# acerbilab/gpyreg

Hardware: AMD Instinct MI355X
Metric: GP-fits/sec (NLL+grad, N=4096 D=10) (higher is better)
Workload: dtype f64

## Files before the change

### gpyreg_amd/_lib.py

```python

from __future__ import annotations

import ctypes as C
import os
import threading

import numpy as np

_HERE = os.path.dirname(os.path.abspath(__file__))
LIB_PATH = os.environ.get("GPYREG_AMD_LIB") or os.path.join(_HERE, "lib", "libgpcore.so")

K_SE, K_MATERN, K_RQ, K_SE_ISO, K_MATERN_ISO = range(5)
F64, F32 = 0, 1
KLO_ZERO, KLO_ROW, KLO_COL = 0, 1, 2
KHI_FULL, KHI_ROW, KHI_COL = 0, 1, 2
CV_LOSSES = {"lpd": 0, "mse": 1}

_dp = C.c_void_p
_ip = C.c_void_p
_vp = C.c_void_p
_dpp = C.POINTER(C.c_double)

SIGNATURES = {
    "gpc_create": (C.c_int, [C.c_int, C.POINTER(_vp)]),
# ... 24 lines not shown
    "gpc_nll_batch_K": (
        C.c_int,
        [_vp, C.c_int, C.c_int, C.c_int, _dp, _vp, _vp, _dp, _dp, C.c_int, C.c_int, _dp, C.c_int, _dp,
         C.c_int, _dp, _dp, _dp, _ip, _ip],
    ),
    "gpc_posterior_batch_K": (
        C.c_int, [_vp, C.c_int, C.c_int, _dp, _dp, _dp, C.c_int, C.POINTER(_vp), _dp, _ip, _ip]),
    "gpc_predict_K": (C.c_int, [_vp, C.c_int, _dp, _dp, _dp, _dp, _dp]),
    "gpc_set_data_gobs": (C.c_int, [_vp, _dp, _dp, C.c_int, C.c_int, _dp, _dp, C.c_int]),
    "gpc_posterior_batch_gobs": (
        C.c_int, [_vp, C.c_int, C.c_int, C.c_int, C.c_int, _dp, _dp, _dp, C.POINTER(_vp), _dp, _dp, _ip, _ip]),
    "gpc_nll_batch_gobs": (C.c_int, [_vp, C.c_int, C.c_int, C.c_int, C.c_int, _dp, _dp, _dp, _dp, _dp, _ip, _ip]),
    "gpc_predict_gobs": (C.c_int, [_vp, _dp, C.c_int, _dp, _dp]),
    "gpc_debug_gobs_cov": (C.c_int, [_vp, C.c_int, C.c_int, _dp, _dp, C.c_int, C.c_int, _dp, C.c_int, _dp]),
    "gpc_debug_gobs_cross": (
        C.c_int, [_vp, C.c_int, C.c_int, _dp, _dp, C.c_int, C.c_int, _dp, C.c_int, _dp, C.c_int, _dp, _dp, _dp]),
    "gpc_post_fetch": (C.c_int, [_vp, C.c_int, _dp, _dp, _dp]),
    "gpc_post_free": (C.c_int, [_vp]),
    "gpc_predict": (C.c_int, [_vp, _dp, C.c_int, _dp, _dp]),
    "gpc_predict_grad": (C.c_int, [_vp, _dp, C.c_int, _dp, _dp, _dp, _dp]),
    "gpc_grad_post": (C.c_int, [_vp, _dp, C.c_int, C.c_int, _dp, _dp, _dp]),
    "gpc_predict_hess": (C.c_int, [_vp, _dp, C.c_int, C.c_int, _dp, _dp, _dp, _dp, _dp, _dp]),
    "gpc_nll_hess": (C.c_int, [_vp, _dp, C.c_int, _dp, C.c_int, C.c_int, _dp, _dp, _dp, _dp]),
    "gpc_cv_grad": (C.c_int, [_vp, C.c_int, _dp, _dp, _dp, _dp, _dp, _dp, _dp]),
    "gpc_predict_hyp_grad": (
        C.c_int, [_vp, _dp, C.c_int, C.c_int, _dp, _dp, C.c_int, C.c_int, _dp, C.c_int, _dp, _dp, _dp, _dp]),
    "gpc_post_append": (C.c_int, [_vp, _dp, _dp, C.c_double, _ip]),
    "gpc_post_recompute": (C.c_int, [_vp, C.c_int, _ip, _dp, _dp, _dp, C.c_int, _dp, _ip, _ip]),
    "gpc_post_append_K": (C.c_int, [_vp, _dp, _dp, _dp, _dp, C.c_double, _ip]),
    "gpc_post_append_block": (C.c_int, [_vp, C.c_int, _dp, _dp, _dp, _ip]),
    "gpc_post_append_block_K": (C.c_int, [_vp, C.c_int, _dp, _dp, _dp, _dp, _dp, _ip]),
    "gpc_post_remove": (C.c_int, [_vp, C.c_int, _ip, _dp, _ip]),
    "gpc_debug_remove_panel": (C.c_int, [_vp, C.c_int, C.c_int, _dp, _dp, _dp, _dp]),
    "gpc_debug_remove_apply": (C.c_int, [_vp, C.c_int, C.c_int, C.c_int, C.c_int, C.c_int, _dp, _dp, _dp]),
    "gpc_post_recompute_K": (C.c_int, [_vp, C.c_int, _ip, _dp, _dp, _dp, C.c_int, _dp, _ip, _ip]),
    "gpc_predict_full": (C.c_int, [_vp, _dp, C.c_int, _dp, _dp]),
    "gpc_predict_cov": (C.c_int, [_vp, _dp, C.c_int, _dp, C.c_int, _dp, C.c_int, _dp, _dp, _dp]),
    "gpc_lookahead_batch": (C.c_int, [_vp, _dp, C.c_int, _dp, C.c_int, _dp, C.c_int, _dp, C.c_int, _ip, _dp]),
    "gpc_draw": (C.c_int, [_vp, _dp, C.c_int, C.c_int, C.c_ulonglong, C.c_int, _dp, _dp, _dp]),
    "gpc_paths_create": (C.c_int, [_vp, C.c_int, C.c_int, C.c_ulonglong, C.c_int, _dp, _dp, C.POINTER(_vp)]),
    "gpc_paths_eval": (C.c_int, [_vp, _dp, C.c_int, _dp, _dp]),
    "gpc_paths_free": (C.c_int, [_vp]),
    "gpc_debug_paths_fetch": (C.c_int, [_vp, C.c_int, _dp, _dp, _dp, _dp]),
    "gpc_quad": (C.c_int, [_vp, _dp, _dp, C.c_int, C.c_int, _dp, _dp]),
    "gpc_quad_grad": (C.c_int, [_vp, _dp, _dp, C.c_int, C.c_int, _dp, _dp, _dp, _dp, _dp, _dp]),
    "gpc_quad_cov": (C.c_int, [_vp, _dp, _dp, C.c_int, _dp, _dp]),
    "gpc_quad_mix": (C.c_int, [_vp, _dp, _dp, _dp, C.c_int, C.c_int, C.c_int] + [_dp] * 10),
    "gpc_cv": (C.c_int, [_vp, C.c_int, _ip, _ip, _dp, _dp, _dp, _dp, _ip]),
    "gpc_last_timing": (C.c_int, [_vp, _dp, _dp]),
    "gpc_last_lauum_timing": (C.c_int, [_vp, _dp, _dp]),
    "gpc_set_option": (C.c_int, [_vp, C.c_char_p, C.c_int]),
    "gpc_get_option": (C.c_int, [_vp, C.c_char_p, _ip]),
    "gpc_mfma_peak": (C.c_int, [_vp, C.c_int, _dp, _dp, _dp]),
    "gpc_debug_gemm": (
        C.c_int,
        [_vp, C.c_int, C.c_int, C.c_int, C.c_int, C.c_int, C.c_int, C.c_double, C.c_int, C.c_int,
         C.c_int, C.c_int, _dp, _dp, _dp],
    ),
    "gpc_debug_leaf": (C.c_int, [_vp, C.c_int, _dp, _dp, _dp, _dp, _ip]),
    "gpc_debug_factor": (C.c_int, [_vp, C.c_int, C.c_int, _dp, _dp, _dp, _dp, _dp, _ip]),
    "gpc_debug_factor_plan": (C.c_int, [_vp] + [C.c_int] * 7 + [_dp] * 7 + [_ip]),
    "gpc_debug_cov": (
        C.c_int,
        [_vp, C.c_int, C.c_int, C.c_int, C.c_int, _dp, C.c_double, C.c_double, _dp, _dp, C.c_int, C.c_int, _dp,
         C.c_int, _dp, _dp, _dp, _dp, _dp],
    ),
    "gpc_debug_blas1": (C.c_int, [_vp, C.c_int, C.c_int, _ip, _vp, _vp, _vp, _vp]),
    "gpc_debug_block_gram": (C.c_int, [_vp, C.c_int, C.c_int, C.c_int, C.c_int, _dp, _dp, C.c_int, _dp]),
    "gpc_debug_hess_contract": (
        C.c_int, [_vp, C.c_int, C.c_int, C.c_int, _dp, _dp, C.c_int, C.c_int, _dp, C.c_int, _dp, _dp, _dp, _dp]),
    "gpc_debug_hyp_cross": (
        C.c_int, [_vp, C.c_int, C.c_int, _dp, _dp, C.c_int, C.c_int, _dp, C.c_int, _dp, _dp, C.c_int, _dp, _dp]),
    "gpc_debug_nll_plane": (
        C.c_int, [_vp, C.c_int, C.c_int, _dp, _dp, C.c_int, C.c_int, C.c_int, _dp, _dp, _dp, _dp, _dp]),
    "gpc_debug_nll_d2": (C.c_int, [_vp, C.c_int, C.c_int, _dp, _dp, C.c_int, C.c_int, _dp, _dp, _dp]),
    "gpc_debug_nll_gram": (C.c_int, [_vp, C.c_int, C.c_int, _dp, _dp]),
    "gpc_debug_cv_trace": (C.c_int, [_vp, C.c_int, C.c_int, _dp, _dp, C.c_int, C.c_int, _dp, _dp, _dp, _dp, _dp]),
    "gpc_debug_cv_weights": (C.c_int, [_vp, C.c_int, C.c_int, _dp, _dp, _dp, _dp, _dp]),
    "gpc_debug_normals": (C.c_int, [_vp, C.c_ulonglong, C.c_int, C.c_int, C.c_int, C.c_int, C.c_int, _dp]),
    "gpc_debug_workspace_hash": (C.c_int, [_vp, C.c_int, C.c_int, C.c_int, _vp]),
    "gpc_debug_chunk_plan": (C.c_int, [C.c_int, C.c_ulonglong, C.c_ulonglong, C.c_ulonglong, C.c_int]),
    "gpc_debug_scratch_bytes": (C.c_int, [C.c_char_p, C.c_int, _ip, C.c_int, _vp, _vp, _ip]),
    "gpc_debug_gemm_queues": (C.c_int, [C.c_int] * 8 + [_ip] * 4),
    "gpc_debug_gemm_form": (
        C.c_int,
        [_vp, C.c_int, C.c_int, C.c_int, C.c_int, C.c_int, C.c_int, _vp, _vp, _dp, C.c_longlong, _dp, _dp, _ip, _ip],
    ),
}
EXPERIMENT_SIGNATURES = {
    "gpc_debug_dag": (C.c_int, [C.c_int, C.c_int, C.c_int, C.c_int, _ip, _ip, _dp, _ip, C.c_int, C.c_int]),
}
EXPERIMENTS_LIB_PATH = os.path.join(_HERE, "lib", "libgpcore_exp.so")

DK_PLANE_FN = C.CFUNCTYPE(C.c_int, _vp, C.c_int, C.c_int, _dpp)


class _GemmProductStruct(C.Structure):
    _fields_ = ([(n, C.c_int) for n in ("M", "N", "K", "a_kmajor", "b_kmajor", "beta", "klo", "khi", "lower_only",
                                        "lda", "ldb", "ldc")]
                + [(n, C.c_longlong) for n in ("off_a", "off_b", "off_c", "s_a", "s_b", "s_c", "size_a", "size_b",
                                               "size_c")]
                + [("alpha", C.c_double), ("A", _vp), ("B", _vp), ("C", _vp)])


class GemmProduct:

    def __init__(self, A, B, C, M, N, K, a_kmajor=0, b_kmajor=0, alpha=1.0, beta=0, klo=0, khi=0, lower_only=0,
                 lda=None, ldb=None, ldc=None, off_a=0, off_b=0, off_c=0, s_a=0, s_b=0, s_c=0):
        self.A, self.B, self.C = _f64(A).ravel(), _f64(B).ravel(), _f64(C).ravel()
        self.M, self.N, self.K = int(M), int(N), int(K)
        self.a_kmajor, self.b_kmajor = int(bool(a_kmajor)), int(bool(b_kmajor))
        self.alpha, self.beta, self.klo, self.khi, self.lower_only = float(alpha), int(beta), klo, khi, int(bool(lower_only))
        self.lda = int(lda if lda is not None else (M if a_kmajor else K))
        self.ldb = int(ldb if ldb is not None else (N if b_kmajor else K))
        self.ldc = int(ldc if ldc is not None else N)
        self.off_a, self.off_b, self.off_c = int(off_a), int(off_b), int(off_c)
        self.s_a, self.s_b, self.s_c = int(s_a), int(s_b), int(s_c)


BLAS1 = {name: code for code, name in enumerate((
    "trmv", "trmv_low", "gemv_sub", "trmv_t_part", "trmv_t_part_low", "trmv_t_sum", "dot", "mat_t_vec", "grad_tail",
    "colsum_prod", "colsum_vec", "diagq", "trace_plane", "extract", "neg_sym", "pad_load", "pad_rect", "load_K",
    "rect_copy", "grow_copy", "append_row", "append_low"))}
BLAS1_GUARD = 128

FORMS = {"plain": 0, "persist": 1, "persist_reserved": 2, "dual": 3, "colsq": 4, "wsq": 5}

_lib = None
_lock = threading.RLock()


def load():
    global _lib
    with _lock:
        if _lib is None:
            if not os.path.exists(LIB_PATH):
                raise RuntimeError(
                    f"{LIB_PATH} is missing: the HIP extension has not been built "
                    "(run `python -c 'import __graft_entry__ as g; g.build()'`). "
                    "gpyreg_amd has no CPU fallback."
                )
            lib = C.CDLL(LIB_PATH)
            for name, (res, args) in SIGNATURES.items():
                fn = getattr(lib, name)
                fn.restype = res
                fn.argtypes = args
            for name, (res, args) in EXPERIMENT_SIGNATURES.items():
                fn = getattr(lib, name, None)
                if fn is not None:
                    fn.restype = res
                    fn.argtypes = args
            _lib = lib
    return _lib


def is_experiments_build() -> bool:
    return hasattr(load(), "gpc_debug_dag")


def _f64(a):
    return np.ascontiguousarray(a, dtype=np.float64)


def _ptr(a):
    if a is None:
        return None
# ... 939 lines not shown
            ptr[1:] = np.cumsum([len(f) for f in folds])
            idx = np.ascontiguousarray(np.concatenate([np.asarray(f).ravel() for f in folds]), dtype=np.int32)
        n_out = F if F else N
        quad, logdet = np.empty((n_out, S)), np.empty((n_out, S))
        info = np.empty((n_out, S), dtype=np.int32)
        rc = self.ctx._lib.gpc_cv(self._h, F, _ptr(ptr), _ptr(idx), _ptr(dmu), _ptr(s2), _ptr(quad), _ptr(logdet),
                                  _ptr(info))
        self.ctx._check(rc, "gpc_cv")
        return dmu, s2, quad, logdet, info

    @_serial
    def free(self):
        if self._h:
            self.ctx._lib.gpc_post_free(self._h)
            self._h = None

    def __del__(self):
        try:
            if self.ctx._h:
                self.free()
        except Exception:
            pass


class Paths:

    def __init__(self, ctx: Context, h, S: int, N: int, D: int, R: int, F: int):
        self.ctx, self._h, self.S, self.N, self.D, self.R, self.F = ctx, h, S, N, D, R, F

    @_serial
    def eval(self, x_star, compute_grad=False):
        if not self._h:
            raise ValueError("paths: the handle has been closed")
        xs = _f64(x_star)
        if xs.ndim != 2 or xs.shape[1] != self.D:
            raise ValueError(f"paths: x_star must be (M, {self.D}), got {xs.shape}")
        M = xs.shape[0]
        f = np.empty((M, self.R, self.S))
        df = np.empty((M, self.D, self.R, self.S)) if compute_grad else None
        rc = self.ctx._lib.gpc_paths_eval(self._h, _ptr(xs), M, _ptr(f), _ptr(df))
        self.ctx._check(rc, "gpc_paths_eval")
        return (f, df) if compute_grad else f

    @_serial
    def fetch(self, s):
        theta, b = np.empty((self.F, self.D)), np.empty(self.F)
        wt, v = np.empty((self.F, self.R)), np.empty((self.N, self.R))
        rc = self.ctx._lib.gpc_debug_paths_fetch(self._h, int(s), _ptr(theta), _ptr(b), _ptr(wt), _ptr(v))
        self.ctx._check(rc, "gpc_debug_paths_fetch")
        return theta, b, wt, v

    @_serial
    def free(self):
        if self._h:
            self.ctx._lib.gpc_paths_free(self._h)
            self._h = None

    def __del__(self):
        try:
            if self.ctx._h:
                self.free()
        except Exception:
            pass


def gemm_queues(ntiles, batch, flags, tiles_m=0, tiles_n=0, klo=0, khi=0, lower_only=0, want_tiles=False,
                want_xcd=False):
    lib = load()
    n = int(ntiles) * int(batch)
    q_total = np.zeros(8, dtype=np.int32)
    q_items = np.full((max(n, 1), 2), -1, dtype=np.int32)
    tiles = np.full((ntiles, 2), -1, dtype=np.int32) if want_tiles else None
    xcd = np.full((batch, ntiles, 2), -1, dtype=np.int32) if want_xcd else None
    rc = lib.gpc_debug_gemm_queues(int(ntiles), int(batch), int(flags), int(tiles_m), int(tiles_n), int(klo), int(khi),
                                   int(bool(lower_only)), q_total.ctypes.data, q_items.ctypes.data, _ptr(tiles),
                                   _ptr(xcd))
    if rc != 0:
        raise RuntimeError(f"gpc_debug_gemm_queues failed (rc={rc})")
    ends = np.concatenate([[0], np.cumsum(np.minimum(q_total, n))])
    queues = [q_items[ends[q]:ends[q + 1]].copy() for q in range(8)]
    return queues, q_total, tiles, xcd


_contexts = {}


def default_device() -> int:
    return int(os.environ.get("GPYREG_AMD_DEVICE", os.environ.get("LOCAL_RANK", "0")))


def context(device: int | None = None) -> Context:
    dev = default_device() if device is None else int(device)
    with _lock:
        ctx = _contexts.get(dev)
        if ctx is None or ctx._h is None:
            ctx = Context(dev)
            _contexts[dev] = ctx
    return ctx
```

### gpyreg_amd/csrc/gemm.h

```cpp
#pragma once
#include "common.h"

#include <type_traits>

namespace gpc {

template <typename T>
constexpr int BKT_v = sizeof(T) == 4 ? 32 : 16;
template <typename T>
constexpr bool MM_SWZ = sizeof(T) == 4;
template <typename T>
constexpr int LDQ_v = MM_SWZ<T> ? BKT_v<T> : BKT_v<T> + 1;
constexpr int ldp_of(int BT) { return BT + 16; }
template <typename T>
constexpr int opsz_of(int BT) {
  return BKT_v<T> * (BT + 16) > BT * LDQ_v<T> ? BKT_v<T> * (BT + 16) : BT * LDQ_v<T>;
}

enum { KLO_ZERO = 0, KLO_ROW = 1, KLO_COL = 2 };
enum { KHI_FULL = 0, KHI_ROW = 1, KHI_COL = 2 };

struct GemmArgs {
  const void* A;
  const void* B;
  void* C;
  long long sA, sB, sC;
  int lda, ldb, ldc;
  int M, N, K;
  double alpha;
  int beta;
  int klo, khi, lower_only;
  int tiles_m, tiles_n;
  int flags = 0;
  const unsigned short* rsv = nullptr;
  int* ctr = nullptr;
  int ntiles = 0, batch = 0;
  double* colsq = nullptr;
  const double* ep_w = nullptr;
  long long ep_sw = 0;
  const double* ep_alpha = nullptr;
};
inline int g_gemm_flags = 8 | 16;

template <typename T, bool KM, int BT, int NT>
__device__ __forceinline__ unsigned stage_toff(int ld, int t) {
  constexpr int VEC = MM<T>::VEC;
  if constexpr (!KM) {
    constexpr int TPR = BKT_v<T> / VEC;
    return (unsigned)(t / TPR) * (unsigned)ld + (unsigned)((t % TPR) * VEC);
  } else {
    constexpr int VPR = BT / VEC;
    return (unsigned)(t / VPR) * (unsigned)ld + (unsigned)((t % VPR) * VEC);
  }
}
template <typename T, bool KM, int BT, int NT>
__device__ __forceinline__ size_t stage_pstride(int ld) {
  constexpr int VEC = MM<T>::VEC;
  if constexpr (!KM)
    return (size_t)(NT / (BKT_v<T> / VEC)) * ld;
  else
    return (size_t)(NT / (BT / VEC)) * ld;
}
template <typename T, bool KM, int BT, int NT, int AUX = 0>
__device__ __forceinline__ void g2r(typename MM<T>::vec_t (&r)[(BT * BKT_v<T>) / (NT * MM<T>::VEC)],
                                    __amdgpu_buffer_rsrc_t rs, unsigned soff, unsigned pstride_bytes,
                                    unsigned voff) {
  using vec_t = typename MM<T>::vec_t;
  constexpr int NV = (BT * BKT_v<T>) / (NT * MM<T>::VEC);
  static_assert(sizeof(vec_t) == 16, "16-byte staging vectors");
  static_assert(KM ? (NT % (BT / MM<T>::VEC) == 0) : (NT % (BKT_v<T> / MM<T>::VEC) == 0), "pass layout");
#pragma unroll
  for (int p = 0; p < NV; ++p) {
    const u32x4 v = __builtin_amdgcn_raw_buffer_load_b128(rs, voff, soff + p * pstride_bytes, AUX);
    r[p] = *reinterpret_cast<const vec_t*>(&v);
  }
}

template <typename T, bool KM, int BT, int NT>
__device__ __forceinline__ void r2s(T* __restrict__ s,
                                    const typename MM<T>::vec_t (&r)[(BT * BKT_v<T>) / (NT * MM<T>::VEC)],
                                    int t) {
  using vec_t = typename MM<T>::vec_t;
  constexpr int VEC = MM<T>::VEC;
  constexpr int NV = (BT * BKT_v<T>) / (NT * VEC);
  constexpr int LDP = ldp_of(BT);
  if constexpr (!KM) {
    constexpr int TPR = BKT_v<T> / VEC;
    constexpr int RPP = NT / TPR;
#pragma unroll
    for (int p = 0; p < NV; ++p) {
      const int row = t / TPR + p * RPP;
      const int kc = (t % TPR) * VEC;
      if constexpr (MM_SWZ<T>) {
        *reinterpret_cast<vec_t*>(s + row * LDQ_v<T> + (((t % TPR) ^ ((row >> 1) & 7)) * VEC)) = r[p];
      } else {
#pragma unroll
        for (int e = 0; e < VEC; ++e) s[row * LDQ_v<T> + kc + e] = r[p][e];
      }
    }
  } else {
    constexpr int VPR = BT / VEC;
#pragma unroll
    for (int p = 0; p < NV; ++p) {
      const int v = t + NT * p;
      const int k = v / VPR;
      const int mc = (v % VPR) * VEC;
      *reinterpret_cast<vec_t*>(s + k * LDP + mc) = r[p];
    }
  }
}

template <typename T, bool KM, int BT>
__device__ __forceinline__ T frag(const T* __restrict__ s, int r0, int kk, int lane) {
  if constexpr (!KM) {
    if constexpr (MM_SWZ<T>) {
      constexpr int VEC = MM<T>::VEC;
      const int k = kk + (lane >> 4), l15 = lane & 15;
      return s[(r0 + l15) * LDQ_v<T> + (((k / VEC) ^ ((l15 >> 1) & 7)) * VEC) + (k % VEC)];
    } else {
      return s[(r0 + (lane & 15)) * LDQ_v<T> + kk + (lane >> 4)];
    }
  }
  else
    return s[(kk + (lane >> 4)) * ldp_of(BT) + r0 + (lane & 15)];
}

__host__ __device__ __forceinline__ void tri_tile(int tile, int& ti, int& tj) {
  int i = (int)((sqrtf(8.f * (float)tile + 1.f) - 1.f) * 0.5f);
  while (i * (i + 1) / 2 > tile) --i;
  while ((i + 1) * (i + 2) / 2 <= tile) ++i;
  ti = i;
  tj = tile - i * (i + 1) / 2;
}

template <bool SQUARE = true>
__host__ __device__ __forceinline__ void tile_of_bx(int klo, int khi, int lower_only, int tiles_m, int tiles_n, int bx,
                                                    int& ti, int& tj) {
  if (lower_only) {
    if constexpr (SQUARE) {
      tri_tile(bx, ti, tj);
    } else {
      int i = (int)((sqrtf(4.f * (float)bx + 1.f) - 1.f) * 0.5f);
      while (i * (i + 1) > bx) --i;
      while ((i + 1) * (i + 2) <= bx) ++i;
      ti = i;
      tj = bx - i * (i + 1);
    }
  } else if (khi == KHI_COL) {
    tj = tiles_n - 1 - bx / tiles_m;
    ti = bx % tiles_m;
  } else if (klo == KLO_COL) {
    tj = bx / tiles_m;
    ti = bx % tiles_m;
  } else if (khi == KHI_ROW) {
    ti = tiles_m - 1 - bx / tiles_n;
    tj = bx % tiles_n;
  } else {
    ti = bx / tiles_n;
    tj = bx % tiles_n;
  }
}

__host__ __device__ __forceinline__ void xcd_order(int gx, int gy, int& bx, int& by) {
  const int total = gx * gy, per = total >> 3;
  const int L = by * gx + bx;
  if (L < (per << 3)) {
    const int wk = (L & 7) * per + (L >> 3);
    bx = wk % gx;
    by = wk / gx;
  }
}

#ifdef GPC_TILE_TRACE
__device__ unsigned long long g_tile_trace[2][4];
#define TILE_TS(k) do { if (HO && threadIdx.x == 0) { const long long _n = wall_clock64(); atomicAdd(&g_tile_trace[BT == 64][k], (unsigned long long)(_n - _ts)); _ts = _n; } } while (0)
#else
#define TILE_TS(k) do { } while (0)
#endif
template <typename T, bool AKM, bool BKM, int BT, int NW, int HO = 0, int EPI = 0, int BTN = BT>
__device__ __forceinline__ void gemm_tile(const GemmArgs& g, const int bx, const int by, T* __restrict__ smem) {
#ifdef GPC_TILE_TRACE
  long long _ts = wall_clock64();
  if (HO && threadIdx.x == 0) atomicAdd(&g_tile_trace[BT == 64][3], 1ull);
#endif
  using acc_t = typename MM<T>::acc_t;
  using vec_t = typename MM<T>::vec_t;
  constexpr int NT = 64 * NW;
  constexpr int NVA = (BT * BKT_v<T>) / (NT * MM<T>::VEC), NVB = (BTN * BKT_v<T>) / (NT * MM<T>::VEC);
  constexpr int OPSZA = opsz_of<T>(BT), OPSZB = opsz_of<T>(BTN), STG = OPSZA + OPSZB;
  constexpr int WCOLS = NW / 2;
  constexpr int WTM = BT / 2;
  constexpr int WTN = BTN / WCOLS;
  constexpr int MRM = WTM / 16, MRN = WTN / 16;
  static_assert(NVA >= 1 && NVB >= 1 && MRM >= 1 && MRN >= 1, "tile shape");
  const int t = threadIdx.x;
  const int lane = t & 63, w = t >> 6, wr = w / WCOLS, wc = w % WCOLS;

  static_assert(BTN == BT || BT == 2 * BTN, "lower tiles of a rectangular launch: two tile columns per tile row");
  int ti, tj;
  tile_of_bx<BTN == BT>(g.klo, g.khi, g.lower_only, g.tiles_m, g.tiles_n, bx, ti, tj);
  const int m0 = ti * BT, n0 = tj * BTN;
  const int m128 = (m0 / TILE) * TILE, n128 = (n0 / TILE) * TILE;
  int k0 = g.klo == KLO_ROW ? m128 : (g.klo == KLO_COL ? n128 : 0);
  int k1 = g.khi == KHI_ROW ? m128 + TILE : (g.khi == KHI_COL ? n128 + TILE : g.K);
  if (k1 > g.K) k1 = g.K;
  const int nk = (k1 - k0) / BKT_v<T>;

  const T* __restrict__ A = reinterpret_cast<const T*>(g.A) + (size_t)by * g.sA;
  const T* __restrict__ B = reinterpret_cast<const T*>(g.B) + (size_t)by * g.sB;
  T* __restrict__ C = reinterpret_cast<T*>(g.C) + (size_t)by * g.sC;

  acc_t acc[MRM][MRN];
#pragma unroll
  for (int i = 0; i < MRM; ++i)
#pragma unroll
    for (int j = 0; j < MRN; ++j) acc[i][j] = acc_t{0, 0, 0, 0};
  constexpr bool TWO_LEVEL = sizeof(T) == 4;
  acc_t acc2[TWO_LEVEL ? MRM : 1][TWO_LEVEL ? MRN : 1];
  if constexpr (TWO_LEVEL) {
#pragma unroll
    for (int i = 0; i < MRM; ++i)
#pragma unroll
      for (int j = 0; j < MRN; ++j) acc2[i][j] = acc_t{0, 0, 0, 0};
  }

  if (nk > 0) {
    vec_t ra[NVA], rb[NVB];
    const unsigned toa = stage_toff<T, AKM, BT, NT>(g.lda, t) * (unsigned)sizeof(T),
                   tob = stage_toff<T, BKM, BTN, NT>(g.ldb, t) * (unsigned)sizeof(T);
    const unsigned psa = (unsigned)(stage_pstride<T, AKM, BT, NT>(g.lda) * sizeof(T)),
                   psb = (unsigned)(stage_pstride<T, BKM, BTN, NT>(g.ldb) * sizeof(T));
    const T* pa = AKM ? A + (size_t)k0 * g.lda + m0 : A + (size_t)m0 * g.lda + k0;
    const T* pb = BKM ? B + (size_t)k0 * g.ldb + n0 : B + (size_t)n0 * g.ldb + k0;
    const size_t rowsa = (size_t)BKT_v<T> * g.lda, rowsb = (size_t)BKT_v<T> * g.ldb;
    __amdgpu_buffer_rsrc_t rsa = make_rsrc(pa), rsb = make_rsrc(pb);
    unsigned ua = 0, ub = 0;
    auto next_slab = [&]() {
      if constexpr (AKM) {
        pa += rowsa;
        rsa = make_rsrc(pa);
      } else {
        ua += (unsigned)(BKT_v<T> * sizeof(T));
      }
      if constexpr (BKM) {
        pb += rowsb;
        rsb = make_rsrc(pb);
      } else {
        ub += (unsigned)(BKT_v<T> * sizeof(T));
      }
    };
    constexpr int AUX = HO == 1 ? 16 : 0;
    g2r<T, AKM, BT, NT, AUX>(ra, rsa, ua, psa, toa);
    g2r<T, BKM, BTN, NT, AUX>(rb, rsb, ub, psb, tob);
    r2s<T, AKM, BT, NT>(smem, ra, t);
    r2s<T, BKM, BTN, NT>(smem + OPSZA, rb, t);
    next_slab();
    g2r<T, AKM, BT, NT, AUX>(ra, rsa, ua, psa, toa);
    g2r<T, BKM, BTN, NT, AUX>(rb, rsb, ub, psb, tob);
    __syncthreads();
    TILE_TS(0);

    T af[2][MRM], bf[2][MRN];
    auto load_frags = [&](int set, const T* a_s, const T* b_s, int kk) {
#pragma unroll
      for (int i = 0; i < MRM; ++i) af[set][i] = frag<T, AKM, BT>(a_s, wr * WTM + i * 16, kk, lane);
#pragma unroll
      for (int j = 0; j < MRN; ++j) bf[set][j] = frag<T, BKM, BTN>(b_s, wc * WTN + j * 16, kk, lane);
    };
    auto mfmas = [&](int set) {
#pragma unroll
      for (int i = 0; i < MRM; ++i)
#pragma unroll
        for (int j = 0; j < MRN; ++j) acc[i][j] = MM<T>::mma(af[set][i], bf[set][j], acc[i][j]);
    };
    constexpr int NMEM = NVA + NVB;
    constexpr int PER = (MRM * MRN) / NMEM;
    constexpr int REM = MRM * MRN - PER * NMEM;
    static_assert(PER >= 1, "interleave pattern");
    constexpr int KS = BKT_v<T> / 4;
    static_assert(KS >= 4 && KS % 2 == 0, "fragment sets alternate per k-step and wrap per slab");
    auto slab = [&](auto cur_c, auto wr_c, auto ld_c) {
      constexpr int CUR = decltype(cur_c)::value;
      constexpr bool WR = decltype(wr_c)::value, LD = decltype(ld_c)::value;
      const T* a_s = smem + CUR * STG;
      const T* b_s = a_s + OPSZA;
      T* a_n = smem + (CUR ^ 1) * STG;
#pragma unroll
      for (int ks = 0; ks < KS - 2; ++ks) {
        load_frags((ks + 1) & 1, a_s, b_s, 4 * (ks + 1));
        mfmas(ks & 1);
        __builtin_amdgcn_sched_group_barrier(0x100, MRM + MRN, 0);
        __builtin_amdgcn_sched_group_barrier(0x008, MRM * MRN, 0);
      }
      load_frags(1, a_s, b_s, 4 * (KS - 1));
      mfmas(0);
      if constexpr (WR) {
        r2s<T, AKM, BT, NT>(a_n, ra, t);
        r2s<T, BKM, BTN, NT>(a_n + OPSZA, rb, t);
      }
      __builtin_amdgcn_sched_group_barrier(0x100, MRM + MRN, 0);
#pragma unroll
      for (int q = 0; q < NMEM; ++q) {
        __builtin_amdgcn_sched_group_barrier(0x008, PER, 0);
        if constexpr (WR) __builtin_amdgcn_sched_group_barrier(0x200, 1, 0);
      }
      if constexpr (REM > 0) __builtin_amdgcn_sched_group_barrier(0x008, REM, 0);
      __syncthreads();
      if constexpr (LD) {
        next_slab();
        g2r<T, AKM, BT, NT, AUX>(ra, rsa, ua, psa, toa);
        g2r<T, BKM, BTN, NT, AUX>(rb, rsb, ub, psb, tob);
      }
      if constexpr (WR) load_frags(0, a_n, a_n + OPSZA, 0);
      mfmas(1);
      if constexpr (WR) __builtin_amdgcn_sched_group_barrier(0x100, MRM + MRN, 0);
#pragma unroll
      for (int q = 0; q < NMEM; ++q) {
        __builtin_amdgcn_sched_group_barrier(0x008, PER, 0);
        if constexpr (LD) __builtin_amdgcn_sched_group_barrier(0x020, 1, 0);
      }
      if constexpr (REM > 0) __builtin_amdgcn_sched_group_barrier(0x008, REM, 0);
    };
    using I0 = std::integral_constant<int, 0>;
    using I1 = std::integral_constant<int, 1>;
    load_frags(0, smem, smem + OPSZA, 0);
    int it = 0;
    for (; it + 3 < nk; it += 2) {
      slab(I0{}, std::true_type{}, std::true_type{});
      slab(I1{}, std::true_type{}, std::true_type{});
      if constexpr (TWO_LEVEL) {
#pragma unroll
        for (int i = 0; i < MRM; ++i)
#pragma unroll
          for (int j = 0; j < MRN; ++j) {
            acc2[i][j] += acc[i][j];
            acc[i][j] = acc_t{0, 0, 0, 0};
          }
      }
    }
    slab(I0{}, std::true_type{}, std::false_type{});
    slab(I1{}, std::false_type{}, std::false_type{});
  }

  TILE_TS(1);
  const T alpha = (T)g.alpha;
  if constexpr (EPI == 1) {
    static_assert(NW == 4 && BT == 128 && BTN == BT, "the reduction is laid out for 2 x 2 waves of 64 x 64");
    double cs[MRN];
#pragma unroll
    for (int j = 0; j < MRN; ++j) {
      double sq = 0.0;
#pragma unroll
      for (int i = 0; i < MRM; ++i)
#pragma unroll
        for (int r = 0; r < 4; ++r) {
          double v;
          if constexpr (TWO_LEVEL)
            v = (double)(alpha * (acc[i][j][r] + acc2[i][j][r]));
          else
            v = (double)(alpha * acc[i][j][r]);
          sq = fma(v, v, sq);
        }
      sq += __shfl_xor(sq, 16, 64);
      sq += __shfl_xor(sq, 32, 64);
      cs[j] = sq;
    }
    double* red = reinterpret_cast<double*>(smem);
    __syncthreads();
    if ((lane >> 4) == 0) {
#pragma unroll
      for (int j = 0; j < MRN; ++j) red[wr * BT + wc * WTN + j * 16 + (lane & 15)] = cs[j];
    }
    __syncthreads();
    if (t < BT) g.colsq[((size_t)by * g.tiles_m + ti) * (size_t)g.N + n0 + t] = red[t] + red[BT + t];
    __syncthreads();
    return;
  }
  if constexpr (EPI == 2) {
    static_assert(NW == 4 && BT == 128 && BTN == BT && HO == 0, "the reduction is laid out for 2 x 2 waves of 64 x 64");
    const T al = (T)g.ep_alpha[by];
    const double* __restrict__ wv = g.ep_w + (size_t)by * g.ep_sw;
    double cs[MRN];
#pragma unroll
    for (int j = 0; j < MRN; ++j) cs[j] = 0.0;
#pragma unroll
    for (int i = 0; i < MRM; ++i) {
      T old[MRN][4];
      double wr4[4];
#pragma unroll
      for (int r = 0; r < 4; ++r) wr4[r] = wv[m0 + wr * WTM + i * 16 + MM<T>::row_of(lane, r)];
#pragma unroll
      for (int j = 0; j < MRN; ++j)
#pragma unroll
        for (int r = 0; r < 4; ++r) {
          const int row = m0 + wr * WTM + i * 16 + MM<T>::row_of(lane, r);
          const int col = n0 + wc * WTN + j * 16 + (lane & 15);
          old[j][r] = C[(size_t)row * g.ldc + col];
        }
#pragma unroll
      for (int j = 0; j < MRN; ++j)
#pragma unroll
        for (int r = 0; r < 4; ++r) {
          T v;
          if constexpr (TWO_LEVEL)
            v = al * (acc[i][j][r] + acc2[i][j][r]);
          else
            v = al * acc[i][j][r];
          v += old[j][r];
          const double d = (double)v;
          cs[j] = fma(wr4[r] * d, d, cs[j]);
        }
    }
#pragma unroll
    for (int j = 0; j < MRN; ++j) {
      cs[j] += __shfl_xor(cs[j], 16, 64);
      cs[j] += __shfl_xor(cs[j], 32, 64);
    }
    double* red = reinterpret_cast<double*>(smem);
    __syncthreads();
    if ((lane >> 4) == 0) {
#pragma unroll
      for (int j = 0; j < MRN; ++j) red[wr * BT + wc * WTN + j * 16 + (lane & 15)] = cs[j];
    }
    __syncthreads();
    if (t < BT) g.colsq[((size_t)by * g.tiles_m + ti) * (size_t)g.N + n0 + t] = red[t] + red[BT + t];
    __syncthreads();
    return;
  }
#pragma unroll
  for (int i = 0; i < MRM; ++i) {
    T old[MRN][4];
    if (g.beta) {
#pragma unroll
      for (int j = 0; j < MRN; ++j)
#pragma unroll
        for (int r = 0; r < 4; ++r) {
          const int row = m0 + wr * WTM + i * 16 + MM<T>::row_of(lane, r);
          const int col = n0 + wc * WTN + j * 16 + (lane & 15);
          if constexpr (HO == 1)
            old[j][r] = __hip_atomic_load(&C[(size_t)row * g.ldc + col], __ATOMIC_RELAXED, __HIP_MEMORY_SCOPE_AGENT);
          else
            old[j][r] = C[(size_t)row * g.ldc + col];
        }
    }
#pragma unroll
    for (int j = 0; j < MRN; ++j)
#pragma unroll
      for (int r = 0; r < 4; ++r) {
        const int row = m0 + wr * WTM + i * 16 + MM<T>::row_of(lane, r);
        const int col = n0 + wc * WTN + j * 16 + (lane & 15);
        T v;
        if constexpr (TWO_LEVEL)
          v = alpha * (acc[i][j][r] + acc2[i][j][r]);
        else
          v = alpha * acc[i][j][r];
        if (g.beta) v += old[j][r];
        if constexpr (HO)
          __hip_atomic_store(&C[(size_t)row * g.ldc + col], v, __ATOMIC_RELAXED, __HIP_MEMORY_SCOPE_AGENT);
        else
          C[(size_t)row * g.ldc + col] = v;
      }
  }
  TILE_TS(2);
}

template <typename T, bool AKM, bool BKM, int BT, int NW, int EPI = 0, int BTN = BT>
__global__ __launch_bounds__(64 * NW, NW / 2) void gemm_kernel(GemmArgs g) {
  __shared__ __attribute__((aligned(16))) T smem[2 * (opsz_of<T>(BT) + opsz_of<T>(BTN))];
  int bx = blockIdx.x, by = blockIdx.y;
  if ((g.flags & 16) && gridDim.y >= 8) {
    xcd_order((int)gridDim.x, (int)gridDim.y, bx, by);
  }
  gemm_tile<T, AKM, BKM, BT, NW, 0, EPI, BTN>(g, bx, by, smem);
}

template <typename T, bool A1, bool B1, bool A2, bool B2, int BT, int NW>
__global__ __launch_bounds__(64 * NW, NW / 2) void gemm_dual_kernel(GemmArgs g1, GemmArgs g2, int n1) {
  __shared__ __attribute__((aligned(16))) T smem[4 * opsz_of<T>(BT)];
  int bx = blockIdx.x, by = blockIdx.y;
  if ((g1.flags & 16) && gridDim.y >= 8) xcd_order((int)gridDim.x, (int)gridDim.y, bx, by);
  if (bx < n1)
    gemm_tile<T, A1, B1, BT, NW>(g1, bx, by, smem);
  else
    gemm_tile<T, A2, B2, BT, NW>(g2, bx - n1, by, smem);
}

template <typename T, bool AKM, bool BKM, int BT, int NW, int EPI = 0>
__global__ __launch_bounds__(64 * NW, NW / 2) void gemm_persist_kernel(GemmArgs g) {
  __shared__ __attribute__((aligned(16))) T smem[4 * opsz_of<T>(BT)];
  __shared__ int next_tile;
  if (g.rsv && cu_reserve_bail(g.rsv, g.ctr)) return;
  if (!(g.flags & 8)) {
    const int total = g.ntiles * g.batch;
    for (;;) {
      if (threadIdx.x == 0) next_tile = atomicAdd(g.ctr, 1);
      __syncthreads();
      const int idx = __builtin_amdgcn_readfirstlane(next_tile);
      __syncthreads();
      if (idx >= total) break;
      gemm_tile<T, AKM, BKM, BT, NW, 0, EPI>(g, idx / g.batch, idx % g.batch, smem);
    }
    return;
  }
  unsigned xcc;
  asm volatile("s_getreg_b32 %0, hwreg(HW_REG_XCC_ID)" : "=s"(xcc));
  const int q0 = (int)(xcc & (NQ - 1));
  const int nclass = g.batch >= NQ ? 1 : NQ / g.batch;
  for (int a = 0; a < NQ; ++a) {
    const int q = (q0 + a) & (NQ - 1);
    int nsq, cls = 0, smp = q;
    if (g.batch >= NQ) {
      nsq = (g.batch - q + NQ - 1) / NQ;
    } else {
      if (q >= g.batch * nclass) continue;
      nsq = 1;
      smp = q % g.batch;
      cls = q / g.batch;
    }
    if (nsq <= 0) continue;
    const int total = ((g.ntiles - cls + nclass - 1) / nclass) * nsq;
    for (;;) {
      if (threadIdx.x == 0) next_tile = atomicAdd(g.ctr + q, 1);
      __syncthreads();
      const int idx = __builtin_amdgcn_readfirstlane(next_tile);
      __syncthreads();
      if (idx >= total) break;
      const int ntq = total / nsq;
      const int sq = idx / ntq, tq = idx - sq * ntq;
      gemm_tile<T, AKM, BKM, BT, NW, 0, EPI>(g, cls + tq * nclass, smp + NQ * sq, smem);
    }
  }
}

inline int queue_nclass(int batch) { return batch >= NQ ? 1 : NQ / batch; }
inline int queue_of(int batch, int nclass, int q, int& cls, int& smp) {
  int nsq;
  cls = 0;
  smp = q;
  if (batch >= NQ) {
    nsq = (batch - q + NQ - 1) / NQ;
  } else {
    if (q >= batch * nclass) return 0;
    nsq = 1;
    smp = q % batch;
    cls = q / batch;
  }
  return nsq;
}
inline int queue_total(int ntiles, int nclass, int cls, int nsq) { return ((ntiles - cls + nclass - 1) / nclass) * nsq; }
inline void queue_item(int total, int nsq, int nclass, int cls, int smp, int idx, int& tile, int& sample) {
  const int ntq = total / nsq;
  const int sq = idx / ntq, tq = idx - sq * ntq;
  tile = cls + tq * nclass;
  sample = smp + NQ * sq;
}
inline void flat_queue_item(int batch, int idx, int& tile, int& sample) {
  tile = idx / batch;
  sample = idx % batch;
}

inline int g_persist_spare = 0;
inline long long g_gemm_launches = 0;
inline int g_block_slots = 512;
template <typename T, int BT, int NW>
inline hipError_t launch_gemm_bt(hipStream_t st, GemmArgs g, bool akm, bool bkm, int batch, int* ctr = nullptr,
                                 const unsigned short* reserve = nullptr) {
  const int tm = g.M / BT, tn = g.N / BT;
  g.tiles_m = tm;
  g.tiles_n = tn;
  g.flags = g_gemm_flags;
  const int ntiles = g.lower_only ? tm * (tm + 1) / 2 : tm * tn;
  if (ntiles <= 0 || batch <= 0) return hipSuccess;
  ++g_gemm_launches;
  g.ntiles = ntiles;
  g.batch = batch;
  g.ctr = ctr;
  const unsigned dyn = 0u;
  const int cap = (BT == 128 ? g_block_slots : 2 * g_block_slots) - g_persist_spare;
  g.rsv = reserve;
  if (ctr && (BT == 128 || reserve) && cap > 0 && ((long long)ntiles * batch > cap || reserve)) {
    dim3 grid(reserve ? (BT == 128 ? cap + 96 : cap) : cap), block(64 * NW);
    if (!akm && !bkm)
      hipLaunchKernelGGL((gemm_persist_kernel<T, false, false, BT, NW>), grid, block, dyn, st, g);
    else if (!akm && bkm)
      hipLaunchKernelGGL((gemm_persist_kernel<T, false, true, BT, NW>), grid, block, dyn, st, g);
    else if (akm && bkm)
      hipLaunchKernelGGL((gemm_persist_kernel<T, true, true, BT, NW>), grid, block, dyn, st, g);
    else
      hipLaunchKernelGGL((gemm_persist_kernel<T, true, false, BT, NW>), grid, block, dyn, st, g);
    return hipGetLastError();
  }
  dim3 grid(ntiles, batch), block(64 * NW);
  if (!akm && !bkm)
    hipLaunchKernelGGL((gemm_kernel<T, false, false, BT, NW>), grid, block, dyn, st, g);
  else if (!akm && bkm)
    hipLaunchKernelGGL((gemm_kernel<T, false, true, BT, NW>), grid, block, dyn, st, g);
  else if (akm && bkm)
    hipLaunchKernelGGL((gemm_kernel<T, true, true, BT, NW>), grid, block, dyn, st, g);
  else
    hipLaunchKernelGGL((gemm_kernel<T, true, false, BT, NW>), grid, block, dyn, st, g);
  return hipGetLastError();
}

#ifdef GPC_EXPERIMENTS
template <typename T>
inline hipError_t launch_gemm_rect(hipStream_t st, GemmArgs g, bool akm, bool bkm, int batch) {
  constexpr int BT = 128, BTN = 64;
  g.tiles_m = g.M / BT;
  g.tiles_n = g.N / BTN;
  g.flags = g_gemm_flags;
  const int ntiles = g.lower_only ? g.tiles_m * (g.tiles_m + 1) : g.tiles_m * g.tiles_n;
  if (ntiles <= 0 || batch <= 0) return hipSuccess;
  ++g_gemm_launches;
  g.ntiles = ntiles;
  g.batch = batch;
  g.ctr = nullptr;
  g.rsv = nullptr;
  dim3 grid(ntiles, batch), block(256);
  if (!akm && !bkm)
    hipLaunchKernelGGL((gemm_kernel<T, false, false, BT, 4, 0, BTN>), grid, block, 0, st, g);
  else if (!akm && bkm)
    hipLaunchKernelGGL((gemm_kernel<T, false, true, BT, 4, 0, BTN>), grid, block, 0, st, g);
  else if (akm && bkm)
    hipLaunchKernelGGL((gemm_kernel<T, true, true, BT, 4, 0, BTN>), grid, block, 0, st, g);
  else
    hipLaunchKernelGGL((gemm_kernel<T, true, false, BT, 4, 0, BTN>), grid, block, 0, st, g);
  return hipGetLastError();
}
template <typename T>
inline hipError_t launch_gemm_w8(hipStream_t st, GemmArgs g, bool akm, bool bkm, int batch) {
  constexpr int BT = 128;
  g.tiles_m = g.M / BT;
  g.tiles_n = g.N / BT;
  g.flags = g_gemm_flags;
  const int ntiles = g.lower_only ? g.tiles_m * (g.tiles_m + 1) / 2 : g.tiles_m * g.tiles_n;
  if (ntiles <= 0 || batch <= 0) return hipSuccess;
  ++g_gemm_launches;
  g.ntiles = ntiles;
  g.batch = batch;
  g.ctr = nullptr;
  g.rsv = nullptr;
  dim3 grid(ntiles, batch), block(512);
  if (!akm && !bkm)
    hipLaunchKernelGGL((gemm_kernel<T, false, false, BT, 8>), grid, block, 0, st, g);
  else if (!akm && bkm)
    hipLaunchKernelGGL((gemm_kernel<T, false, true, BT, 8>), grid, block, 0, st, g);
  else if (akm && bkm)
    hipLaunchKernelGGL((gemm_kernel<T, true, true, BT, 8>), grid, block, 0, st, g);
  else
    hipLaunchKernelGGL((gemm_kernel<T, true, false, BT, 8>), grid, block, 0, st, g);
  return hipGetLastError();
}
inline int g_rect_min_blocks = 0;
inline int g_rect_mode = 0;

#else
constexpr int g_rect_min_blocks = 0;
#endif

inline int g_small_launch_blocks = 1100;
inline bool g_dual_launch = true;
template <typename T>
inline hipError_t launch_gemm(hipStream_t st, GemmArgs g, bool akm, bool bkm, int batch, int force_bt = 0,
                             int* ctr = nullptr, const unsigned short* reserve = nullptr, int reserved_small_bt = 128) {
  const int tm = g.M / TILE, tn = g.N / TILE;
  const long long blocks128 = (long long)(g.lower_only ? tm * (tm + 1) / 2 : tm * tn) * batch;
  const bool small = force_bt ? (force_bt == 64) : (blocks128 < g_small_launch_blocks);
#ifdef GPC_EXPERIMENTS
  if ((force_bt == 12864 || (!force_bt && small && g_rect_min_blocks > 0 && blocks128 >= g_rect_min_blocks)) && !(reserve && ctr))
    return (g_rect_mode == 1 && force_bt != 12864) ? launch_gemm_w8<T>(st, g, akm, bkm, batch) : launch_gemm_rect<T>(st, g, akm, bkm, batch);
#endif
  if (small && !(reserve && ctr)) return launch_gemm_bt<T, 64, 4>(st, g, akm, bkm, batch);
#ifdef GPC_EXPERIMENTS
  if (small && reserved_small_bt == 64) return launch_gemm_bt<T, 64, 4>(st, g, akm, bkm, batch, ctr, reserve);
#endif
// ... 84 lines not shown
```

### gpyreg_amd/csrc/gpcore.hip

```cpp
#include "../../include/gpcore.h"

#include <algorithm>
#include <atomic>
#include <chrono>
#include <cmath>
#include <cstdlib>
#include <cstring>
#include <memory>
#include <mutex>

#include "blas1.h"
#include "block_append.h"
#include "common.h"
#include "covfun.h"
#include "cv.h"
#include "cvgrad.h"
#include "draw.h"
#include "gemm.h"
#include "gradobs.h"
#include "gradpost.h"
#include "hess.h"
#include "hypgrad.h"
#include "nll_hess.h"
#include "leaf.h"
// ... 291 lines not shown
    up_fallback.clear();
    if (zero_bytes % 8) {
      hipError_t e = hipMemsetAsync(zero, 0, zero_bytes, st);
      if (e != hipSuccess) return e;
      zero_bytes = 0;
    }
    upd.zero = zero;
    upd.zero8 = zero_bytes / 8;
    if (upd.nseg == 0 && upd.zero8 == 0 && !upd.xs && !upd.r_out && !upd.dvec_out) return hipSuccess;
    const unsigned long long words = gathered_bytes / 8 + upd.zero8 + (upd.xs ? (unsigned long long)upd.npad * upd.D * upd.cnt : 0ull) +
                                     ((upd.r_out || upd.dvec_out) ? (unsigned long long)upd.fnpad * upd.fcnt : 0ull);
    const int blocks = (int)std::min<unsigned long long>(256, (words + 255) / 256);
    hipLaunchKernelGGL(xfer_kernel, dim3(std::max(1, blocks)), dim3(256), 0, st, upd);
    upd.nseg = 0;
    return hipGetLastError();
  }
  hipError_t take_up(hipStream_t st, void* zero, size_t zero_bytes, XferDesc& out) {
    for (Pending& q : up_fallback) {
      hipError_t e = up(q.dst, q.src, q.n, st);
      if (e != hipSuccess) return e;
    }
    up_fallback.clear();
    if (zero_bytes % 8) {
      hipError_t e = hipMemsetAsync(zero, 0, zero_bytes, st);
      if (e != hipSuccess) return e;
      zero_bytes = 0;
    }
    upd.zero = zero;
    upd.zero8 = zero_bytes / 8;
    out = upd;
    upd.nseg = 0;
    return hipSuccess;
  }
  bool down_plain = false;
  hipError_t gather(void* dst, const void* src, size_t n, hipStream_t st) {
    if (n == 0) return hipSuccess;
    void* h = (n % 8 == 0 && downd.nseg < XferDesc::MAXSEG && n <= kGather / 8) ? alloc(n) : nullptr;
    if (!h) {
      down_plain = true;
      return hipMemcpyAsync(dst, src, n, hipMemcpyDeviceToHost, st);
    }
    pend.push_back({dst, h, n});
    downd.seg[downd.nseg++] = {h, src, (unsigned long long)(n / 8)};
    return hipSuccess;
  }
  hipError_t flush_down(hipStream_t st, unsigned long long* flag = nullptr, unsigned long long seq = 0, int* done_ctr = nullptr) {
    if (downd.nseg == 0) return hipSuccess;
    unsigned long long words = 0;
    for (int k = 0; k < downd.nseg; ++k) words += downd.seg[k].n8;
    int blocks = (int)std::min<unsigned long long>(64, (words + 255) / 256);
    if (flag && !done_ctr) blocks = 1;
    downd.flag = flag;
    downd.seq = seq;
    downd.done_ctr = done_ctr;
    hipLaunchKernelGGL(xfer_kernel, dim3(std::max(1, blocks)), dim3(256), 0, st, downd);
    downd.nseg = 0;
    downd.flag = nullptr;
    return hipGetLastError();
  }
  void release() {
    for (Blk& b : blks) (void)hipHostFree(b.p);
    blks.clear();
    pend.clear();
  }
};

}

struct gpc_ctx {
  int device = 0;
  hipStream_t st = nullptr;
  hipEvent_t ev[4] = {nullptr, nullptr, nullptr, nullptr};
  static constexpr int MAXG = 8;
  hipStream_t gst[MAXG] = {};
  hipStream_t sst[MAXG + 1] = {};
  static constexpr int NDEV = 64;
  hipEvent_t dev_ev[MAXG + 1][NDEV] = {};
  hipEvent_t ev_bfork[MAXG + 1] = {}, ev_btail[MAXG + 1] = {};
  int defer_min = -1, defer_reserve = 8;
  unsigned cu_seen[64] = {};
  bool cu_map_ok = false;
  DevBuf rsv_tbl;
  int nll_block = -1;
  int solves_beside_lauum = 1;
#ifdef GPC_EXPERIMENTS
  int rl_panel = 0;
  int rl_ahead_max = 8;
#endif
  int stable = 0;
  int small_path = 1;
  int small_poll = 1, small_timing = 0;
  double* land_blk = nullptr;
  static constexpr size_t LAND_BYTES = 64u << 10;
  unsigned long long land_seq = 0;
  unsigned long long small_polled = 0, small_synced = 0;
  int last_chunk = 0;
  unsigned long long grad_post_gram_us = 0;
  unsigned long long gobs_cov_us = 0, gobs_cross_us = 0;
  unsigned long long hess_contract_us = 0;
  unsigned long long nll_hess_gram_us = 0, nll_hess_contract_us = 0;
  unsigned long long cv_grad_trace_us = 0;
  unsigned long long lookahead_batch_loop_us = 0;
  unsigned long long cov_fused = 0;
  unsigned long long quad_mix_gemms = 0;
  int check_queues = 0;
  hipEvent_t ev_up = nullptr, ev_done[MAXG] = {};
  int groups = 2;
  hipEvent_t ev_l0[MAXG + 1] = {}, ev_l1[MAXG + 1] = {};
  double ms_lauum = 0, flops_lauum = 0;
  int lauum_groups = 0;
  std::string err;
  std::string devinfo;
  int N = 0, D = 0, npad = 0;
  DevBuf dX;
  DevBuf dY;
  GobsDims gobs;
  DevBuf gpts, gxs;
  std::vector<double> hy;
  DevBuf mA, mW, mT;
  DevBuf xs, spb, mulb, divb;
  DevBuf dvec, rvec, zvec, avec;
  DevBuf tpart;
  DevBuf scal;
  DevBuf parts, gout, diagq;
  DevBuf dmb, dsn2b, mg, ng;
  DevBuf cs, covs;
  DevBuf qmix;
  DevBuf nhs;
  DevBuf lab;
  DevBuf hgs;
  DevBuf dbg1, dbg2, dbg3;
  PinBuf pin;
  struct GraphEntry {
    unsigned long long key[4] = {0, 0, 0, 0};
    unsigned long long epoch = 0;
    hipGraphExec_t exec = nullptr;
    unsigned long long last_use = 0;
    double flops = 0;
  };
  static constexpr int NGRAPH = 16;
  GraphEntry graphs[NGRAPH];
  unsigned long long graph_clock = 0;
  int graph_max_npad = 4096;
  bool capturing = false;
  DevBuf tile_ctr;
  static constexpr int CTR_PER_GROUP = 1024;
  std::vector<DevBuf> pool;
  DevBuf pool_take(size_t need) {
    int best = -1;
    for (int i = 0; i < (int)pool.size(); ++i)
      if (pool[i].bytes >= need && pool[i].bytes <= need + need / 2 &&
          (best < 0 || pool[i].bytes < pool[best].bytes))
        best = i;
    DevBuf r;
    if (best >= 0) {
      r = pool[best];
      pool.erase(pool.begin() + best);
    }
    return r;
  }
  void pool_give(DevBuf& b) {
    if (!b.p) return;
    pool.push_back(b);
    b.p = nullptr;
    b.bytes = 0;
    while (pool.size() > 6) {
// ... 381 lines not shown
    }
    return 0;
  }

  int device_section(hipStream_t st, int off, int n, hipEvent_t f0, hipEvent_t f1, int gidx = gpc_ctx::MAXG) {
    Batch& b = *B;
    const int npad = b.npad, N = b.N, D = b.D;
    T* Ac = A + (size_t)off * sM;
    T* Wc = W + (size_t)off * sM;
    T* Tc = Tm + (size_t)off * sM;
    double* xs = c->xs.as<double>() + (size_t)off * npad * D;
    double* spb = c->spb.as<double>() + (size_t)off * SP_STRIDE;
    double* rvec = c->rvec.as<double>() + (size_t)off * npad;
    double* zvec = c->zvec.as<double>() + (size_t)off * npad;
    double* avec = c->avec.as<double>() + (size_t)off * npad;
    double* d_logdet = c->scal.as<double>() + off;
    double* d_quad = c->scal.as<double>() + chunk_cnt + off;
    int* d_info = reinterpret_cast<int*>(c->scal.as<double>() + 2 * chunk_cnt) + off;
    const int t64 = npad / CT, ntl = t64 * (t64 + 1) / 2;
    split_build = false;
    if (kmode()) {
      HIPCHK(c, c->dbg1.ensure((size_t)N * N * sizeof(double)));
      const size_t gper = (size_t)gobs.P() * D;
      if (gobs.Ng > 0) {
        HIPCHK(c, c->gxs.ensure((size_t)chunk_cnt * gper * sizeof(double)));
        launch_gobs_scale(st, gobs, c->gpts.as<double>(), c->mulb.as<double>() + (size_t)off * D,
                          c->divb.as<double>() + (size_t)off * D, n, c->gxs.as<double>() + (size_t)off * gper);
      }
      for (int i = 0; i < n; ++i) {
        if (gobs.Ng > 0)
          launch_gobs_cov(st, b.cd, gobs, c->gxs.as<double>() + (size_t)(off + i) * gper, spb + (size_t)i * SP_STRIDE,
                          c->mulb.as<double>() + (size_t)(off + i) * D, c->divb.as<double>() + (size_t)(off + i) * D,
                          c->dbg1.as<double>());
        else
          HIPCHK(c, hipMemcpyAsync(c->dbg1.p, Kptr[chunk_s0 + off + i], (size_t)N * N * sizeof(double),
                                   hipMemcpyHostToDevice, st));
        dim3 gl(npad / 64, npad / 4), bl(64, 4);
        hipLaunchKernelGGL((load_K_kernel<T>), gl, bl, 0, st, (const double*)c->dbg1.p, N, npad,
                           (const double*)(spb + (size_t)i * SP_STRIDE),
                           (const double*)(c->dvec.as<double>() + (size_t)(off + i) * npad), Ac + (size_t)i * sM);
      }
    } else {
      if (!prescaled) {
        const long long tot = (long long)npad * D;
        dim3 grid((unsigned)((tot + 255) / 256), n);
        hipLaunchKernelGGL(scale_x_kernel, grid, dim3(256), 0, st, c->dX.as<double>(), N, npad, D,
                           c->mulb.as<double>() + (size_t)off * D, c->divb.as<double>() + (size_t)off * D, xs);
      }
      const int head64 = 1024 / CT, ntl_head = head64 * (head64 + 1) / 2;
      split_build = (defer_node > 0 || use_rl) && !c->capturing && gpc::g_persist_spare >= 0 && npad >= 2048 && reserve_tbl();
      const double* dv = c->dvec.as<double>() + (size_t)off * npad;
      if (split_build) {
        GPC_COV_DISPATCH(build_kernel, T, b.cd, dim3(ntl_head, n), dim3(256), 0, st, b.cd, (const double*)xs,
                         (const double*)spb, dv, N, npad, Ac, sM, npad, 0);
        hipStream_t sd = c->sst[gidx];
        int* bctr = c->tile_ctr.as<int>() + (size_t)gidx * gpc_ctx::CTR_PER_GROUP + gpc_ctx::CTR_PER_GROUP - CTR_STRIDE;
        HIPCHK(c, hipMemsetAsync(bctr, 0, CTR_STRIDE * sizeof(int), st));
        HIPCHK(c, hipEventRecord(c->ev_bfork[gidx], st));
        HIPCHK(c, hipStreamWaitEvent(sd, c->ev_bfork[gidx], 0));
        GPC_COV_DISPATCH(build_persist_kernel, T, b.cd, dim3(4 * gpc::g_block_slots / 2 + 128), dim3(256), 0, sd, b.cd,
                         (const double*)xs, (const double*)spb, dv, N, npad, Ac, sM, npad, ntl_head, ntl, n,
                         reserve_tbl(), bctr);
        HIPCHK(c, hipEventRecord(c->ev_btail[gidx], sd));
      } else {
        GPC_COV_DISPATCH(build_kernel, T, b.cd, dim3(ntl, n), dim3(256), 0, st, b.cd, (const double*)xs,
                         (const double*)spb, dv, N, npad, Ac, sM, npad, 0);
      }
    }
    HIPCHK(c, hipGetLastError());

    if (f0 && !c->capturing) HIPCHK(c, hipEventRecord(f0, st));
    Factor<T> F;
    F.st = st;
    F.batch = n;
    F.npad = npad;
    F.A = Ac;
    F.W = Wc;
    F.Tm = Tc;
    F.sA = F.sW = F.sT = sM;
    F.logdet = d_logdet;
    F.info = d_info;
    F.nvalid = N;
    F.stable = stable || c->stable;
    if ((defer_node > 0 || use_rl) && !c->capturing && gpc::g_persist_spare >= 0) {
      F.side = c->sst[gidx];
      F.evs = c->dev_ev[gidx];
      F.nev = gpc_ctx::NDEV - 2;
      F.defer_min = defer_node;
      F.reserve = reserve_tbl();
    }
#ifdef GPC_EXPERIMENTS
    if (indep_mode && !c->capturing) {
      F.reserve = c->rsv_tbl4.template as<unsigned short>();
      F.reserved_small_bt = 64;
      F.reserve_all = true;
      F.reserve_min = c->indep_min_tiles;
    }
#endif
    if (c->check_queues && !c->capturing) F.qlog = &qlog;
    if (split_build) {
      F.ev_tail = c->ev_btail[gidx];
      F.tail_row0 = 1024;
    }
    if (gpc::g_persist_spare >= 0) {
      F.ctr = c->tile_ctr.as<int>() + (size_t)gidx * gpc_ctx::CTR_PER_GROUP;
      F.ctr_cap = gpc_ctx::CTR_PER_GROUP - CTR_STRIDE;
      const long long tmx = npad / TILE, biggest = tmx * (tmx + 1) / 2 * n;
      if (defer_node > 0 || F.reserve_all || biggest >= std::min<long long>(gpc::g_small_launch_blocks, gpc::g_block_slots - gpc::g_persist_spare))
        HIPCHK(c, hipMemsetAsync(F.ctr, 0, (gpc_ctx::CTR_PER_GROUP - CTR_STRIDE) * sizeof(int), st));
      else
        F.ctr = nullptr;
    }
    const bool full_inv = (mode != MODE_NLL);
    const int nll_blk = c->nll_block >= 0 ? c->nll_block
                                          : (npad >= 2048 ? 512 : 0);
    const bool nll_blocked = !use_rl && mode == MODE_NLL && nll_blk >= TILE && npad > nll_blk;
    bool dag_done = false, dag_has_lauum = false;
    if (nll_blocked) F.nll_block = nll_blk;
#ifdef GPC_EXPERIMENTS
    if (use_dag && !use_rl) {
      int rc = dag_section(st, gidx, F, nll_blocked ? nll_blk : 0, full_inv, dag_has_lauum);
      if (rc < 0) return rc;
      dag_done = rc == 0;
      if (dag_done && getenv("GPC_DAG_SYNC")) {
        (void)hipStreamSynchronize(c->sst[gidx]);
        (void)hipStreamSynchronize(st);
      }
    }
    if (!dag_done && use_rl) {
      F.rl_panel = c->rl_panel;
      F.rl_lookahead = (double)n * std::pow((double)npad / 4096.0, 3.0) <= (double)c->rl_ahead_max;
      F.potrf_rl();
      dag_done = true;
    }
#endif
    if (dag_done) {
    } else if (nll_blocked) {
      F.nll_block = nll_blk;
      F.potrf_nll(0, npad);
    } else {
      F.potrf_inv(0, npad, full_inv, mode == MODE_POST);
    }
    const bool solves_beside_lauum = mode == MODE_GRAD && !c->capturing && !kmode() && c->solves_beside_lauum &&
                                     sizeof(T) == 8 && npad >= 2048 && gpc::g_persist_spare >= 0 && !dag_has_lauum && !indep_mode;
    auto solves = [&](hipStream_t sx) -> int {
      const hipStream_t keep = F.st;
      F.st = sx;
      F.low_regs = sx != st;
#ifdef GPC_EXPERIMENTS
      if (use_rl)
        F.forward_solve_rl(rvec, zvec);
      else
#endif
      if (nll_blocked)
        F.forward_solve_nll(0, npad, rvec, zvec);
      else
        F.forward_solve(0, npad, full_inv, rvec, zvec);
      F.st = keep;
      F.low_regs = false;
      if (mode == MODE_NLL) {
        hipLaunchKernelGGL(dot_kernel, dim3(1, n), dim3(256), 0, sx, (const double*)zvec, (const double*)zvec,
                           npad, npad, d_quad);
      } else {
        double* tpart = c->tpart.as<double>() + (size_t)off * (npad / TRC) * npad;
        const dim3 gt((npad + 64 * MM<T>::VEC - 1) / (64 * MM<T>::VEC), npad / TRC, n);
        if (sx != st)
          hipLaunchKernelGGL((trmv_t_part_low_kernel<T>), gt, dim3(256), 0, sx, (const T*)Wc, sM, npad, (const double*)zvec,
                             npad, tpart, d_quad);
        else
          hipLaunchKernelGGL((trmv_t_part_kernel<T, 8>), gt, dim3(256), 0, sx, (const T*)Wc, sM, npad, (const double*)zvec,
                             npad, tpart, d_quad);
        hipLaunchKernelGGL(trmv_t_sum_kernel, dim3(npad / 128, n), dim3(128), 0, sx, (const double*)tpart, npad,
                           (const double*)spb, (int)SP_STRIDE, (int)SP_SL, avec);
      }
      HIPCHK(c, hipGetLastError());
      return 0;
    };
    hipEvent_t ev_solved = nullptr;
    if (mode == MODE_GRAD) {
      if (solves_beside_lauum) {
        hipStream_t sx = c->sst[gidx];
        hipEvent_t ev_fork = c->dev_ev[gidx][gpc_ctx::NDEV - 1];
        ev_solved = c->dev_ev[gidx][gpc_ctx::NDEV - 2];
        HIPCHK(c, hipEventRecord(ev_fork, st));
        HIPCHK(c, hipStreamWaitEvent(sx, ev_fork, 0));
        if (int rc = solves(sx)) return rc;
        HIPCHK(c, hipEventRecord(ev_solved, sx));
      }
      if (!dag_has_lauum) {
        if (!c->capturing) HIPCHK(c, hipEventRecord(c->ev_l0[gidx], st));
        F.lauum(Tc, sM);
        if (!c->capturing) {
          HIPCHK(c, hipEventRecord(c->ev_l1[gidx], st));
          lauum_n[gidx] = n;
        }
      }
    }
    HIPCHK(c, F.err);
    HIPCHK(c, hipGetLastError());
    if (f1 && !c->capturing) HIPCHK(c, hipEventRecord(f1, st));
    c->last_flops += F.flops;

    if (ev_solved)
      HIPCHK(c, hipStreamWaitEvent(st, ev_solved, 0));
    else if (int rc = solves(st))
      return rc;
    HIPCHK(c, hipGetLastError());

    const int Pn = P();
    if (mode == MODE_GRAD) {
      double* parts = c->parts.as<double>() + (size_t)off * ntl * Pn;
      double* diagq = c->diagq.as<double>() + (size_t)off * npad;
      if (kmode()) {
        hipLaunchKernelGGL((diagq_kernel<T>), dim3(1, n), dim3(256), 0, st, (const T*)Tc, sM, npad, (const double*)avec,
                           (const double*)spb, N, diagq, c->gout.as<double>() + (size_t)off * Pn, Pn);
      } else {
        GPC_COV_DISPATCH(trace_kernel, T, b.cd, dim3(ntl, n), dim3(256), 4 * (((Pn + 3) & ~3) + 4) * sizeof(double), st,
                         b.cd, (const double*)xs, (const double*)spb, (const double*)avec, N, npad, (const T*)Tc, sM,
                         npad, parts, ntl, diagq);
        const int mN = mean_N > 0 ? mean_N : 0, nN = (noise_N > 0 && b.vec_noise) ? noise_N : 0;
        hipLaunchKernelGGL(grad_tail_kernel, dim3(Pn + mN + nN, n), dim3(256), 0, st, (const double*)parts, ntl, Pn,
                           c->gout.as<double>() + (size_t)off * Pn,
                           (mN && dm) ? (const double*)(c->dmb.as<double>() + (size_t)off * N * mean_N) : nullptr, N, mN,
                           (const double*)avec, mN ? c->mg.as<double>() + (size_t)off * mean_N : nullptr,
                           nN ? (const double*)(c->dsn2b.as<double>() + (size_t)off * N * noise_N) : nullptr, nN,
                           (const double*)diagq, nN ? c->ng.as<double>() + (size_t)off * noise_N : nullptr, npad);
        HIPCHK(c, hipGetLastError());
        return 0;
      }
      if (mean_N > 0)
        hipLaunchKernelGGL(mat_t_vec_kernel, dim3(mean_N, n), dim3(256), 0, st,
                           (const double*)(c->dmb.as<double>() + (size_t)off * N * mean_N), N, mean_N,
                           (const double*)avec, npad, c->mg.as<double>() + (size_t)off * mean_N);
      if (noise_N > 0 && b.vec_noise)
        hipLaunchKernelGGL(mat_t_vec_kernel, dim3(noise_N, n), dim3(256), 0, st,
                           (const double*)(c->dsn2b.as<double>() + (size_t)off * N * noise_N), N, noise_N,
                           (const double*)diagq, npad, c->ng.as<double>() + (size_t)off * noise_N);
      HIPCHK(c, hipGetLastError());
    }
    return 0;
  }

#ifdef GPC_EXPERIMENTS
  bool use_dag = false;
  bool indep_mode = false;
  int dag_trace_n = 0;
  bool dag_auto(int cnt, int npad) const { return false; }

  gpc_ctx::DagEntry* dag_plan(int nll_blk, bool full_inv, bool with_lauum, double* flops1) {
    Batch& b = *B;
    const int npad = b.npad;
    const unsigned long long key = (unsigned long long)npad | ((unsigned long long)sizeof(T) << 20) |
                                   ((unsigned long long)nll_blk << 24) | ((unsigned long long)full_inv << 40) |
                                   ((unsigned long long)with_lauum << 41) | ((unsigned long long)mode << 42) |
                                   ((unsigned long long)c->dag_small_tiles << 44) | ((unsigned long long)c->dag_crit_pct << 56);
    for (auto& e : c->dag_cache)
      if (e.key == key) {
        e.last_use = ++c->dag_clock;
        *flops1 = e.plan.work_us;
        return e.plan.ntasks > 0 ? &e : nullptr;
      }
    PlanRecorder rec;
    Factor<T> F;
    F.rec = &rec;
    F.st = nullptr;
    F.batch = 1;
    F.npad = npad;
    F.A = static_cast<T*>(const_cast<void*>(dag_fake_base(0)));
    F.W = static_cast<T*>(const_cast<void*>(dag_fake_base(1)));
    F.Tm = static_cast<T*>(const_cast<void*>(dag_fake_base(2)));
    F.sA = F.sW = F.sT = sM;
    F.nvalid = b.N;
    F.dual_launch = false;
    if (nll_blk > 0) {
// ... 2685 lines not shown
  }
  return 0;
}

template <typename T>
int debug_gemm_impl(gpc_ctx* c, int M, int N, int K, int akm, int bkm, double alpha, int beta, int klo,
                    int khi, int lower, const double* A, const double* B, double* C) {
  if (upload_as<T>(c, c->dbg1, A, (size_t)M * K)) return -1;
  if (upload_as<T>(c, c->dbg2, B, (size_t)N * K)) return -1;
  if (upload_as<T>(c, c->dbg3, C, (size_t)M * N)) return -1;
  GemmArgs g;
  g.A = c->dbg1.p;
  g.B = c->dbg2.p;
  g.C = c->dbg3.p;
  g.sA = g.sB = g.sC = 0;
  g.lda = akm ? M : K;
  g.ldb = bkm ? N : K;
  g.ldc = N;
  g.M = M;
  g.N = N;
  g.K = K;
  g.alpha = alpha;
  g.beta = beta;
  g.klo = klo;
  g.khi = khi;
  g.lower_only = lower & 1;
  g.tiles_n = N / TILE;
  HIPCHK(c, launch_gemm<T>(c->st, g, akm != 0, bkm != 0, 1, (lower & 0x100) ? 64 : ((lower & 0x200) ? 128 : ((lower & 0x400) ? 12864 : 0))));
  return download_as<T>(c, c->dbg3.as<T>(), C, (size_t)M * N);
}

struct HookMem {
  std::vector<void*> ps;
  ~HookMem() {
    for (void* p : ps) (void)hipFree(p);
  }
  hipError_t get(void** p, size_t bytes) {
    hipError_t e = hipMalloc(p, bytes ? bytes : 16);
    if (e == hipSuccess) ps.push_back(*p);
    return e;
  }
};
struct GemmGlobalsGuard {
  const int flags = gpc::g_gemm_flags, slots = gpc::g_block_slots, spare = gpc::g_persist_spare;
  ~GemmGlobalsGuard() {
    gpc::g_gemm_flags = flags;
    gpc::g_block_slots = slots;
    gpc::g_persist_spare = spare;
  }
};

const char* form_product_error(const gpc_gemm_product& p, int batch, int vec) {
  constexpr long long CAP = 1ll << 27;
  if (p.M <= 0 || p.N <= 0 || p.K <= 0 || p.M % TILE || p.N % TILE || p.K % TILE) return "sizes must be multiples of 128";
  if (p.lower_only && p.M != p.N) return "lower_only needs M == N";
  if ((p.beta != 0 && p.beta != 1) || p.klo < 0 || p.klo > 2 || p.khi < 0 || p.khi > 2) return "beta is 0 or 1, klo and khi 0..2";
  if (!p.A || !p.B || !p.C) return "A, B and C are required";
  const long long ra = p.a_kmajor ? p.K : p.M, ca = p.a_kmajor ? p.M : p.K;
  const long long rb = p.b_kmajor ? p.K : p.N, cb = p.b_kmajor ? p.N : p.K;
  struct Op {
    long long rows, cols, ld, off, stride, size;
    bool staged;
  } ops[3] = {{ra, ca, p.lda, p.off_a, p.s_a, p.size_a, true},
              {rb, cb, p.ldb, p.off_b, p.s_b, p.size_b, true},
              {p.M, p.N, p.ldc, p.off_c, p.s_c, p.size_c, false}};
  for (const Op& o : ops) {
    if (o.ld < o.cols || o.off < 0 || o.stride < 0 || o.size <= 0 || o.size > CAP || o.ld > CAP || o.stride > CAP)
      return "leading dimension below the extent, or a negative / oversized offset, stride or allocation";
    const long long span = (o.rows - 1) * o.ld + o.cols;
    if (o.off + (batch - 1) * o.stride + span > o.size) return "an operand reaches past its allocation";
    if (o.staged && (o.ld % vec || o.off % vec || o.stride % vec))
      return "lda, ldb and the offsets and strides of A and B must be multiples of the 16-byte vector";
    if (!o.staged && batch > 1 && o.stride < span) return "the C blocks of two samples overlap";
  }
  return nullptr;
}

template <typename T>
int debug_gemm_form_impl(gpc_ctx* c, int form, int tile, int batch, int flags, int block_slots,
                         const gpc_gemm_product* const* prods, int nprod, const double* ep_w, long long ep_sw,
                         const double* ep_alpha, double* colsq, int* counters, int* available) {
  HookMem mem;
  GemmGlobalsGuard guard;
  if (flags >= 0) gpc::g_gemm_flags = flags;
  if (block_slots > 0) {
    gpc::g_block_slots = block_slots;
    gpc::g_persist_spare = 0;
  }
  const unsigned short* rsv = nullptr;
  if (form == GPC_FORM_PERSIST_RESERVED) {
    rsv = ctx_reserve_tbl(c);
    if (!rsv) {
      *available = 0;
      return 0;
    }
  }
  *available = 1;
  GemmArgs g[2];
  T* dC[2] = {nullptr, nullptr};
  auto up = [&](const double* src, long long n, T** dst) -> int {
    HIPCHK(c, mem.get(reinterpret_cast<void**>(dst), (size_t)n * sizeof(T)));
    if constexpr (sizeof(T) == 8) {
      HIPCHK(c, hipMemcpyAsync(*dst, src, (size_t)n * 8, hipMemcpyHostToDevice, c->st));
      HIPCHK(c, hipStreamSynchronize(c->st));
    } else {
      std::vector<float> tmp((size_t)n);
      for (long long i = 0; i < n; ++i) tmp[(size_t)i] = (float)src[i];
      HIPCHK(c, hipMemcpyAsync(*dst, tmp.data(), (size_t)n * 4, hipMemcpyHostToDevice, c->st));
      HIPCHK(c, hipStreamSynchronize(c->st));
    }
    return 0;
  };
  for (int i = 0; i < nprod; ++i) {
    const gpc_gemm_product& p = *prods[i];
    T *dA = nullptr, *dB = nullptr;
    if (up(p.A, p.size_a, &dA) || up(p.B, p.size_b, &dB) || up(p.C, p.size_c, &dC[i])) return -1;
    GemmArgs& a = g[i];
    a.A = dA + p.off_a;
    a.B = dB + p.off_b;
    a.C = dC[i] + p.off_c;
    a.sA = p.s_a;
    a.sB = p.s_b;
    a.sC = p.s_c;
    a.lda = p.lda;
    a.ldb = p.ldb;
    a.ldc = p.ldc;
    a.M = p.M;
    a.N = p.N;
    a.K = p.K;
    a.alpha = p.alpha;
    a.beta = p.beta;
    a.klo = p.klo;
    a.khi = p.khi;
    a.lower_only = p.lower_only ? 1 : 0;
  }
  int* ctr = nullptr;
  HIPCHK(c, mem.get(reinterpret_cast<void**>(&ctr), CTR_STRIDE * sizeof(int)));
  HIPCHK(c, hipMemsetAsync(ctr, 0, CTR_STRIDE * sizeof(int), c->st));
  const gpc_gemm_product& p0 = *prods[0];
  const size_t ncolsq = (size_t)batch * (p0.M / TILE) * p0.N;
  double* dcolsq = nullptr;
  if (form == GPC_FORM_COLSQ || form == GPC_FORM_WSQ) {
    HIPCHK(c, mem.get(reinterpret_cast<void**>(&dcolsq), ncolsq * sizeof(double)));
    HIPCHK(c, hipMemsetAsync(dcolsq, 0xff, ncolsq * sizeof(double), c->st));
    g[0].colsq = dcolsq;
  }
  if (form == GPC_FORM_WSQ) {
    double *dw = nullptr, *da = nullptr;
    const size_t nw = (size_t)(batch - 1) * ep_sw + p0.M;
    HIPCHK(c, mem.get(reinterpret_cast<void**>(&dw), nw * sizeof(double)));
    HIPCHK(c, mem.get(reinterpret_cast<void**>(&da), (size_t)batch * sizeof(double)));
    HIPCHK(c, hipMemcpyAsync(dw, ep_w, nw * sizeof(double), hipMemcpyHostToDevice, c->st));
    HIPCHK(c, hipMemcpyAsync(da, ep_alpha, (size_t)batch * sizeof(double), hipMemcpyHostToDevice, c->st));
    HIPCHK(c, hipStreamSynchronize(c->st));
    g[0].ep_w = dw;
    g[0].ep_sw = ep_sw;
    g[0].ep_alpha = da;
  }
  const bool akm = p0.a_kmajor != 0, bkm = p0.b_kmajor != 0;
  switch (form) {
    case GPC_FORM_PLAIN:
    case GPC_FORM_PERSIST:
    case GPC_FORM_PERSIST_RESERVED: {
      int* qc = form == GPC_FORM_PLAIN ? nullptr : ctr;
      if (tile == 64)
        HIPCHK(c, (launch_gemm_bt<T, 64, 4>(c->st, g[0], akm, bkm, batch, qc, rsv)));
      else
        HIPCHK(c, (launch_gemm_bt<T, 128, 4>(c->st, g[0], akm, bkm, batch, qc, rsv)));
      break;
    }
    case GPC_FORM_DUAL:
      HIPCHK(c, launch_gemm_dual_small<T>(c->st, g[0], g[1], batch));
      break;
    case GPC_FORM_COLSQ:
      HIPCHK(c, launch_gemm_colsq<T>(c->st, g[0], batch, ctr));
      break;
    default:
      HIPCHK(c, launch_gemm_wsq<T>(c->st, g[0], batch));
      break;
  }
  HIPCHK(c, hipStreamSynchronize(c->st));
  for (int i = 0; i < nprod; ++i)
    if (download_as<T>(c, dC[i], prods[i]->C, (size_t)prods[i]->size_c)) return -1;
  if (dcolsq) HIPCHK(c, hipMemcpy(colsq, dcolsq, ncolsq * sizeof(double), hipMemcpyDeviceToHost));
  HIPCHK(c, hipMemcpy(counters, ctr, NQ * sizeof(int), hipMemcpyDeviceToHost));
  return 0;
}

template <typename T>
int debug_factor_impl(gpc_ctx* c, int n, const double* A, double* L, double* W, double* Ainv,
                      double* logdet, int* info) {
  const int npad = pad_tile(n);
  const size_t msz = (size_t)npad * npad;
  HIPCHK(c, c->mA.ensure(msz * sizeof(T)));
  HIPCHK(c, c->mW.ensure(msz * sizeof(T)));
  HIPCHK(c, c->mT.ensure(msz * sizeof(T)));
  HIPCHK(c, c->dbg1.ensure((size_t)n * n * 8));
  HIPCHK(c, c->scal.ensure(64));
  HIPCHK(c, hipMemcpyAsync(c->dbg1.p, A, (size_t)n * n * 8, hipMemcpyHostToDevice, c->st));
  HIPCHK(c, hipMemsetAsync(c->scal.p, 0, 64, c->st));
  dim3 blk(64, 4), gp(npad / 64, npad / 4);
  hipLaunchKernelGGL((pad_load_kernel<T>), gp, blk, 0, c->st, c->dbg1.as<double>(), n, npad, c->mA.as<T>());
  Factor<T> F;
  F.st = c->st;
  F.batch = 1;
  F.npad = npad;
  F.A = c->mA.as<T>();
  F.W = c->mW.as<T>();
  F.Tm = c->mT.as<T>();
  F.sA = F.sW = F.sT = (long long)msz;
  F.logdet = c->scal.as<double>();
  F.info = reinterpret_cast<int*>(c->scal.as<double>() + 1);
  F.nvalid = n;
  F.potrf_inv(0, npad, true, true);
  HIPCHK(c, F.err);
  HIPCHK(c, hipGetLastError());
  HIPCHK(c, c->dbg3.ensure((size_t)n * n * 8));
  dim3 gn((n + 63) / 64, (n + 3) / 4);
  if (L) {
    hipLaunchKernelGGL((extract_kernel<T>), gn, blk, 0, c->st, (const T*)F.A, npad, n, 0, c->dbg3.as<double>());
    HIPCHK(c, hipMemcpyAsync(L, c->dbg3.p, (size_t)n * n * 8, hipMemcpyDeviceToHost, c->st));
    HIPCHK(c, hipStreamSynchronize(c->st));
  }
  if (W) {
    hipLaunchKernelGGL((extract_kernel<T>), gn, blk, 0, c->st, (const T*)F.W, npad, n, 0, c->dbg3.as<double>());
    HIPCHK(c, hipMemcpyAsync(W, c->dbg3.p, (size_t)n * n * 8, hipMemcpyDeviceToHost, c->st));
    HIPCHK(c, hipStreamSynchronize(c->st));
  }
  if (Ainv) {
    F.lauum(F.Tm, F.sT);
    HIPCHK(c, F.err);
    hipLaunchKernelGGL((extract_kernel<T>), gn, blk, 0, c->st, (const T*)F.Tm, npad, n, 0, c->dbg3.as<double>());
    HIPCHK(c, hipMemcpyAsync(Ainv, c->dbg3.p, (size_t)n * n * 8, hipMemcpyDeviceToHost, c->st));
    HIPCHK(c, hipStreamSynchronize(c->st));
  }
  double h[2];
  HIPCHK(c, hipMemcpyAsync(h, c->scal.p, 16, hipMemcpyDeviceToHost, c->st));
  HIPCHK(c, hipStreamSynchronize(c->st));
  if (logdet) *logdet = h[0];
  if (info) memcpy(info, &h[1], sizeof(int));
  return 0;
}

struct ScratchDev {
  std::vector<void*> ps;
  ~ScratchDev() {
    for (void* p : ps) (void)hipFree(p);
  }
  template <typename U>
  U* get(size_t n) {
    void* p = nullptr;
    if (hipMalloc(&p, std::max<size_t>(n, 1) * sizeof(U)) != hipSuccess) return nullptr;
    ps.push_back(p);
    return static_cast<U*>(p);
  }
};

template <typename T>
int debug_factor_plan_impl(gpc_ctx* c, int npad, int nvalid, int batch, int plan, int nll_block, int flags, double* A,
                           double* W, double* Tm, const double* r, double* z, double* Ainv, double* logdet, int* info) {
  const size_t msz = (size_t)npad * npad, tot = msz * batch, vtot = (size_t)npad * batch;
  ScratchDev sd;
  T* dA = sd.get<T>(tot);
  T* dW = sd.get<T>(tot);
  T* dT = sd.get<T>(tot);
  double* dld = sd.get<double>(batch);
  int* dinfo = sd.get<int>(batch);
  double* dr = r ? sd.get<double>(vtot) : nullptr;
  double* dz = r ? sd.get<double>(vtot) : nullptr;
  if (!dA || !dW || !dT || !dld || !dinfo || (r && (!dr || !dz))) FAIL(c, "gpc_debug_factor_plan: out of device memory");
  auto up = [&](T* dst, const double* src) -> int {
    std::vector<T> h(src, src + tot);
    HIPCHK(c, hipMemcpy(dst, h.data(), tot * sizeof(T), hipMemcpyHostToDevice));
    return 0;
  };
  if (up(dA, A) || up(dW, W) || up(dT, Tm)) return -1;
  HIPCHK(c, hipMemsetAsync(dld, 0, batch * sizeof(double), c->st));
  HIPCHK(c, hipMemsetAsync(dinfo, 0, batch * sizeof(int), c->st));
  if (r) {
    HIPCHK(c, hipMemcpyAsync(dr, r, vtot * 8, hipMemcpyHostToDevice, c->st));
    HIPCHK(c, hipMemsetAsync(dz, 0xff, vtot * 8, c->st));
  }
  Factor<T> F;
  F.st = c->st;
  F.batch = batch;
  F.npad = npad;
  F.nvalid = nvalid;
  F.A = dA;
  F.W = dW;
  F.Tm = dT;
  F.sA = F.sW = F.sT = (long long)msz;
  F.logdet = dld;
  F.info = dinfo;
  F.stable = (flags & 1) != 0;
  const bool keep_L = (flags & 2) != 0;
  if (plan == 2) {
    F.nll_block = nll_block;
    F.potrf_nll(0, npad);
  } else {
    F.potrf_inv(0, npad, plan == 0, keep_L);
  }
  HIPCHK(c, F.err);
  HIPCHK(c, hipGetLastError());
  if (r) {
    if (plan == 2)
      F.forward_solve_nll(0, npad, dr, dz);
    else
      F.forward_solve(0, npad, plan == 0, dr, dz);
    HIPCHK(c, hipGetLastError());
  }
  HIPCHK(c, hipStreamSynchronize(c->st));
  if (download_as<T>(c, dA, A, tot) || download_as<T>(c, dW, W, tot) || download_as<T>(c, dT, Tm, tot)) return -1;
  if (r) HIPCHK(c, hipMemcpy(z, dz, vtot * 8, hipMemcpyDeviceToHost));
  HIPCHK(c, hipMemcpy(logdet, dld, batch * sizeof(double), hipMemcpyDeviceToHost));
  HIPCHK(c, hipMemcpy(info, dinfo, batch * sizeof(int), hipMemcpyDeviceToHost));
  if (flags & 4) {
    F.lauum(F.Tm, F.sT);
    HIPCHK(c, F.err);
    HIPCHK(c, hipGetLastError());
    if (download_as<T>(c, dT, Ainv, tot)) return -1;
  }
  return 0;
}

template <typename T>
int debug_cov_impl(gpc_ctx* c, int which, CovDesc cd, const double* hyp, double kscale, double sl, const double* dvec,
                   const double* X, int N, const double* Xstar, int M, const double* mat, const double* vec,
                   double* out0, double* out1, double* xs_out) {
  hipStream_t st = c->st;
  const int D = cd.D, npad = pad_tile(N), mpad = M > 0 ? pad_tile(M) : 0, Pn = cd.cov_N + 1;
  const int t64 = npad / CT, ntl = t64 * (t64 + 1) / 2;
  std::vector<double> mul(D), dv(D), sp(SP_STRIDE, 0.0), hd(npad, 1.0), hv(npad, 0.0);
  double sf2 = 0.0, rqa = 1.0;
  scaling_of(cd.kind, cd.degree, D, hyp, mul.data(), dv.data(), &sf2, &rqa);
  sp[SP_SF2] = sf2;
  sp[SP_RQA] = rqa;
  sp[SP_KSCALE] = kscale;
  sp[SP_SL] = sl;
  if (dvec) std::copy(dvec, dvec + N, hd.begin());
  if (vec) std::copy(vec, vec + N, hv.begin());
  ScratchDev sd;
  double* dX = sd.get<double>((size_t)N * D);
  double* dmul = sd.get<double>(D);
  double* ddv = sd.get<double>(D);
  double* dsp = sd.get<double>(SP_STRIDE);
  double* dd = sd.get<double>(npad);
  double* dvv = sd.get<double>(npad);
  double* xs = sd.get<double>((size_t)npad * D);
  if (!dX || !dmul || !ddv || !dsp || !dd || !dvv || !xs) FAIL(c, "gpc_debug_cov: out of device memory");
  HIPCHK(c, hipMemcpyAsync(dX, X, (size_t)N * D * 8, hipMemcpyHostToDevice, st));
  HIPCHK(c, hipMemcpyAsync(dmul, mul.data(), (size_t)D * 8, hipMemcpyHostToDevice, st));
  HIPCHK(c, hipMemcpyAsync(ddv, dv.data(), (size_t)D * 8, hipMemcpyHostToDevice, st));
  HIPCHK(c, hipMemcpyAsync(dsp, sp.data(), SP_STRIDE * 8, hipMemcpyHostToDevice, st));
  HIPCHK(c, hipMemcpyAsync(dd, hd.data(), (size_t)npad * 8, hipMemcpyHostToDevice, st));
  HIPCHK(c, hipMemcpyAsync(dvv, hv.data(), (size_t)npad * 8, hipMemcpyHostToDevice, st));
  const long long tot = (long long)npad * D;
  if (which != 1)
    hipLaunchKernelGGL(scale_x_kernel, dim3((unsigned)((tot + 255) / 256), 1), dim3(256), 0, st, (const double*)dX, N, npad,
                       D, (const double*)dmul, (const double*)ddv, xs);
  const size_t msz = (size_t)npad * npad;
  if (which == 0 || which == 1) {
    T* A = sd.get<T>(msz);
    if (!A) FAIL(c, "gpc_debug_cov: out of device memory");
    HIPCHK(c, hipMemsetAsync(A, 0, msz * sizeof(T), st));
    if (which == 0) {
      GPC_COV_DISPATCH(build_kernel, T, cd, dim3(ntl, 1), dim3(256), 0, st, cd, (const double*)xs, (const double*)dsp,
                       (const double*)dd, N, npad, A, (long long)msz, npad, 0);
    } else {
      XferDesc u{};
      u.nseg = 0;
      u.X = dX;
      u.mul = dmul;
      u.dv = ddv;
      u.xs = xs;
      u.n = N;
      u.npad = npad;
      u.D = D;
// ... 3087 lines not shown
  bool singletons = true;
  if (F > 0) {
    if (fold_ptr[0] != 0) FAIL(c, "gpc_cv: fold_ptr must start at 0");
    std::vector<int> owner(N, -1);
    for (int f = 0; f < F; ++f) {
      const int lo = fold_ptr[f], k = fold_ptr[f + 1] - lo;
      const std::string name = "gpc_cv: fold " + std::to_string(f);
      if (k <= 0) FAIL(c, name + " is empty");
      if (k >= N) FAIL(c, name + " holds all " + std::to_string(N) + " points: nothing is left to predict from");
      singletons = singletons && k == 1;
      for (int j = 0; j < k; ++j) {
        const int i = fold_idx[lo + j];
        if (i < 0 || i >= N)
          FAIL(c, name + " has index " + std::to_string(i) + " out of range [0, " + std::to_string(N) + ")");
        if (j > 0 && i <= fold_idx[lo + j - 1]) FAIL(c, name + " is unsorted: its indices must ascend strictly");
        if (owner[i] >= 0)
          FAIL(c, name + " overlaps fold " + std::to_string(owner[i]) + " at index " + std::to_string(i));
        owner[i] = f;
      }
    }
  }
  if (int rc = require_factorized(po, "gpc_cv")) return rc;
  HIPCHK(c, hipSetDevice(c->device));
  const bool f64 = po->dtype == GPC_F64;
  if (F == 0) return f64 ? cv_loo_impl<double>(po, dmu, s2, quad, logdet, info) : cv_loo_impl<float>(po, dmu, s2, quad, logdet, info);
  if (!singletons)
    return f64 ? cv_fold_impl<double>(po, F, fold_ptr, fold_idx, dmu, s2, quad, logdet, info)
               : cv_fold_impl<float>(po, F, fold_ptr, fold_idx, dmu, s2, quad, logdet, info);
  const size_t ns = (size_t)N * S;
  std::vector<double> tm_(ns), ts(ns), tq(ns), tl(ns);
  std::vector<int> ti(ns);
  if (int rc = f64 ? cv_loo_impl<double>(po, tm_.data(), ts.data(), tq.data(), tl.data(), ti.data())
                   : cv_loo_impl<float>(po, tm_.data(), ts.data(), tq.data(), tl.data(), ti.data()))
    return rc;
  std::fill(dmu, dmu + ns, std::nan(""));
  std::fill(s2, s2 + ns, std::nan(""));
  for (int f = 0; f < F; ++f) {
    const size_t i = (size_t)fold_idx[fold_ptr[f]];
    for (int s = 0; s < S; ++s) {
      dmu[i * S + s] = tm_[i * S + s];
      s2[i * S + s] = ts[i * S + s];
      if (quad) quad[(size_t)f * S + s] = tq[i * S + s];
      if (logdet) logdet[(size_t)f * S + s] = tl[i * S + s];
      if (info) info[(size_t)f * S + s] = ti[i * S + s];
    }
  }
  return 0;
}

int gpc_last_timing(gpc_ctx* c, double* ms_total, double* ms_factor) {
  if (!c) return -2;
  if (ms_total) *ms_total = c->ms_total;
  if (ms_factor) *ms_factor = c->ms_factor;
  return 0;
}

namespace {
struct Option {
  const char* name;
  int (*get)(gpc_ctx*);
  int (*set)(gpc_ctx*, int);
};
#ifdef GPC_EXPERIMENTS
constexpr int IS_EXPERIMENTS_BUILD = 1;
#else
constexpr int IS_EXPERIMENTS_BUILD = 0;
#endif
int clamp_to(int lo, int hi, int v) { return std::max(lo, std::min(hi, v)); }
int tile_multiple(int v) { return std::max(TILE, (v / TILE) * TILE); }
int engine_choice(int v) { return v == 1 || v == 2 ? v : 0; }
#define GPC_GET(expr) [](gpc_ctx* c) -> int { (void)c; return (int)(expr); }
#define GPC_SET(stmt) [](gpc_ctx* c, int v) -> int { (void)c; stmt; return 0; }
#define GPC_COUNTER(field) GPC_GET(c->field & 0x7fffffff), nullptr
const Option OPTIONS[] = {
    {"groups", GPC_GET(c->groups), GPC_SET(c->groups = clamp_to(1, gpc_ctx::MAXG, v))},
    {"small_blocks", GPC_GET(gpc::g_small_launch_blocks), GPC_SET(gpc::g_small_launch_blocks = v)},
    {"dual_launch", GPC_GET(gpc::g_dual_launch ? 1 : 0), GPC_SET(gpc::g_dual_launch = v != 0)},
    {"leaf", GPC_GET(gpc::g_leaf_version), GPC_SET(gpc::g_leaf_version = v == 3 ? 3 : 5)},
    {"defer_min", GPC_GET(c->defer_min), GPC_SET(c->defer_min = v)},
    {"defer_reserve", GPC_GET(c->defer_reserve), [](gpc_ctx* c, int v) -> int { return c->defer_reserve = v, build_reserve_table(c); }},
    {"leaf_fault", nullptr, GPC_SET(gpc::g_leaf_fault = v != 0)},
    {"nll_block", GPC_GET(c->nll_block), GPC_SET(c->nll_block = v < 0 ? -1 : (v == 0 ? 0 : tile_multiple(v)))},
    {"solves_beside_lauum", GPC_GET(c->solves_beside_lauum), GPC_SET(c->solves_beside_lauum = v != 0)},
    {"stable", GPC_GET(c->stable), GPC_SET(c->stable = v != 0)},
    {"small_path", GPC_GET(c->small_path), GPC_SET(c->small_path = v != 0)},
    {"check_queues", GPC_GET(c->check_queues), GPC_SET(c->check_queues = v != 0)},
    {"small_poll", GPC_GET(c->small_poll), GPC_SET(c->small_poll = v != 0)},
    {"small_timing", GPC_GET(c->small_timing), GPC_SET(c->small_timing = v != 0)},
    {"small_polled", GPC_COUNTER(small_polled)},
    {"small_synced", GPC_COUNTER(small_synced)},
    {"hess_contract_us", GPC_COUNTER(hess_contract_us)},
    {"nll_hess_gram_us", GPC_COUNTER(nll_hess_gram_us)},
    {"nll_hess_contract_us", GPC_COUNTER(nll_hess_contract_us)},
    {"cv_grad_trace_us", GPC_COUNTER(cv_grad_trace_us)},
    {"gobs_cov_us", GPC_COUNTER(gobs_cov_us)},
    {"gobs_cross_us", GPC_COUNTER(gobs_cross_us)},
    {"grad_post_gram_us", GPC_COUNTER(grad_post_gram_us)},
    {"lookahead_batch_loop_us", GPC_COUNTER(lookahead_batch_loop_us)},
    {"cov_fused", GPC_COUNTER(cov_fused)},
    {"quad_mix_gemms", GPC_COUNTER(quad_mix_gemms)},
    {"start_mult_log10", nullptr, GPC_SET(c->start_mult = std::pow(10.0, clamp_to(0, 9, v)))},
    {"append_fail_mask", nullptr, GPC_SET(c->append_fail_mask = (unsigned)v)},
    {"block_engine", GPC_GET(c->block_engine), GPC_SET(c->block_engine = engine_choice(v))},
    {"block_engine_ran", GPC_GET(c->block_engine_ran), nullptr},
    {"paths_engine", GPC_GET(c->paths_engine), GPC_SET(c->paths_engine = engine_choice(v))},
    {"paths_engine_ran", GPC_GET(c->paths_engine_ran), nullptr},
    {"paths_solve_engine", GPC_GET(c->paths_solve_engine), GPC_SET(c->paths_solve_engine = engine_choice(v))},
    {"paths_solve_engine_ran", GPC_GET(c->paths_solve_engine_ran), nullptr},
    {"cv_engine", GPC_GET(c->cv_engine), GPC_SET(c->cv_engine = engine_choice(v))},
    {"cv_engine_ran", GPC_GET(c->cv_engine_ran), nullptr},
    {"block_appended", GPC_COUNTER(block_appended)},
    {"block_stale", GPC_COUNTER(block_stale)},
    {"remove_fail_mask", nullptr, GPC_SET(c->remove_fail_mask = (unsigned)v)},
    {"remove_force", GPC_GET(c->remove_force), GPC_SET(c->remove_force = v != 0)},
    {"remove_max_panels", GPC_GET(c->remove_force ? (1 << 30) : RM_SWEEP_MAX_PANELS), nullptr},
    {"remove_min_rows", GPC_GET(c->remove_force ? 0 : RM_MIN_KEPT_ROWS), nullptr},
    {"removed", GPC_COUNTER(points_removed)},
    {"remove_stale", GPC_COUNTER(remove_stale)},
    {"last_chunk", GPC_GET(c->last_chunk), nullptr},
    {"experiments", GPC_GET(IS_EXPERIMENTS_BUILD), nullptr},
};
#ifdef GPC_EXPERIMENTS
#define GPC_INT_OPTION(name, lvalue, clamped) {name, GPC_GET(lvalue), GPC_SET(lvalue = (clamped))}
const Option EXPERIMENT_OPTIONS[] = {
    GPC_INT_OPTION("rect_min", gpc::g_rect_min_blocks, v),
    GPC_INT_OPTION("rect_mode", gpc::g_rect_mode, v != 0),
    GPC_INT_OPTION("indep", c->indep, v),
    GPC_INT_OPTION("indep_max", c->indep_max, clamp_to(2, gpc_ctx::MAXG, v)),
    GPC_INT_OPTION("indep_min_tiles", c->indep_min_tiles, std::max(1, v)),
    GPC_INT_OPTION("rl_ahead_max", c->rl_ahead_max, v),
    GPC_INT_OPTION("rl_panel", c->rl_panel, v <= 0 ? 0 : tile_multiple(v)),
    GPC_INT_OPTION("dag", c->dag, v),
    GPC_INT_OPTION("dag_small_tiles", c->dag_small_tiles, v),
    GPC_INT_OPTION("dag_lauum", c->dag_lauum, v),
    GPC_INT_OPTION("dag_leaf_blocks", c->dag_leaf_blocks, v),
    GPC_INT_OPTION("dag_aborts", c->dag_aborts, v),
    GPC_INT_OPTION("dag_runs", c->dag_runs, v),
    GPC_INT_OPTION("dag_urgent_cus", c->dag_urgent_cus, clamp_to(0, 15, v)),
    GPC_INT_OPTION("dag_gate", c->dag_gate, v),
    GPC_INT_OPTION("dag_gate_pct", c->dag_gate_pct, clamp_to(0, 100, v)),
    GPC_INT_OPTION("dag_crit_pct", c->dag_crit_pct, clamp_to(0, 100, v)),
    GPC_INT_OPTION("dag_timeout_ms", c->dag_timeout_ms, std::max(1, v)),
};
#undef GPC_INT_OPTION
#endif
#undef GPC_GET
#undef GPC_SET
#undef GPC_COUNTER

const Option* find_option(const char* name) {
  for (const Option& o : OPTIONS)
    if (!strcmp(o.name, name)) return &o;
#ifdef GPC_EXPERIMENTS
  for (const Option& o : EXPERIMENT_OPTIONS)
    if (!strcmp(o.name, name)) return &o;
#endif
  return nullptr;
}
}

int gpc_set_option(gpc_ctx* c, const char* name, int value) {
  if (!c || !name) return -2;
  const Option* o = find_option(name);
  if (!o || !o->set) FAIL(c, "gpc_set_option: unknown option");
  if (o->set(c, value)) return -1;
  ++g_alloc_epoch;
// ... 70 lines not shown
            hipLaunchKernelGGL((mfma_peak_kernel<float, 4>), dim3(blocks), dim3(256), 0, c->st, c->dbg1.as<float>(), iters, d_clk);
          else
            hipLaunchKernelGGL((mfma_peak_kernel<float, 16>), dim3(blocks), dim3(256), 0, c->st, c->dbg1.as<float>(), iters, d_clk);
        }
      };
      launch();
      HIPCHK(c, hipStreamSynchronize(c->st));
      HIPCHK(c, hipEventRecord(c->ev[0], c->st));
      const int reps = 4;
      for (int r = 0; r < reps; ++r) launch();
      HIPCHK(c, hipEventRecord(c->ev[1], c->st));
      HIPCHK(c, hipStreamSynchronize(c->st));
      float ms = 0;
      HIPCHK(c, hipEventElapsedTime(&ms, c->ev[0], c->ev[1]));
      const double flops = (double)reps * blocks * 4.0 * iters * nacc * (2.0 * 16 * 16 * 4);
      const double tf = flops / (ms * 1e-3) / 1e12;
      long long hclk[2] = {0, 0};
      HIPCHK(c, hipMemcpy(hclk, d_clk, sizeof hclk, hipMemcpyDeviceToHost));
      if (tf > best) {
        best = tf;
        best_ghz = hclk[1] > 0 ? (double)hclk[0] / ((double)hclk[1] * 10.0) : 0.0;
        best_cyc = best_ghz * 1e9 * (4.0 * prop.multiProcessorCount) * (2.0 * 16 * 16 * 4) / (tf * 1e12);
      }
    }
  *tflops = best;
  if (cycles_per_mfma) *cycles_per_mfma = best_cyc;
  if (clock_ghz) *clock_ghz = best_ghz;
  return 0;
}


int gpc_debug_gemm(gpc_ctx* c, int dtype, int M, int N, int K, int a_kmajor, int b_kmajor, double alpha,
                   int beta, int klo, int khi, int lower_only, const double* A, const double* B, double* C) {
  if (!c) return -2;
  if (M % TILE || N % TILE || K % TILE || M <= 0 || N <= 0 || K <= 0) FAIL(c, "gpc_debug_gemm: sizes must be multiples of 128");
  if ((lower_only & 1) && M != N) FAIL(c, "gpc_debug_gemm: lower_only needs M == N");
#ifndef GPC_EXPERIMENTS
  if (lower_only & 0x400) FAIL(c, "gpc_debug_gemm: the rectangular tile exists in the experiments build only");
#endif
  HIPCHK(c, hipSetDevice(c->device));
  return dtype == GPC_F64
             ? debug_gemm_impl<double>(c, M, N, K, a_kmajor, b_kmajor, alpha, beta, klo, khi, lower_only, A, B, C)
             : debug_gemm_impl<float>(c, M, N, K, a_kmajor, b_kmajor, alpha, beta, klo, khi, lower_only, A, B, C);
}

int gpc_debug_gemm_queues(int ntiles, int batch, int flags, int tiles_m, int tiles_n, int klo, int khi, int lower_only,
                          int* q_total, int* q_items, int* tile_ij, int* xcd_items) {
  if (ntiles <= 0 || batch <= 0 || !q_total || (long long)ntiles * batch > (1ll << 24)) return -2;
  for (int q = 0; q < NQ; ++q) q_total[q] = 0;
  int* out = q_items;
  if (!(flags & 8)) {
    q_total[0] = ntiles * batch;
    for (int idx = 0; out && idx < q_total[0]; ++idx, out += 2) flat_queue_item(batch, idx, out[0], out[1]);
  } else {
    const int nclass = queue_nclass(batch);
    for (int q = 0; q < NQ; ++q) {
      int nsq, cls, smp;
      nsq = queue_of(batch, nclass, q, cls, smp);
      if (nsq <= 0) continue;
      q_total[q] = queue_total(ntiles, nclass, cls, nsq);
      for (int idx = 0; out && idx < q_total[q]; ++idx, out += 2) {
        if (out - q_items >= 2ll * ntiles * batch) return -3;
        queue_item(q_total[q], nsq, nclass, cls, smp, idx, out[0], out[1]);
      }
    }
  }
  if (tile_ij) {
    if (tiles_m <= 0 || tiles_n <= 0 || klo < 0 || klo > 2 || khi < 0 || khi > 2) return -2;
    if (ntiles != (lower_only ? tiles_m * (tiles_m + 1) / 2 : tiles_m * tiles_n)) return -2;
    for (int bx = 0; bx < ntiles; ++bx) tile_of_bx(klo, khi, lower_only, tiles_m, tiles_n, bx, tile_ij[2 * bx], tile_ij[2 * bx + 1]);
  }
  if (xcd_items) {
    for (int by = 0; by < batch; ++by)
      for (int bx = 0; bx < ntiles; ++bx) {
        int x = bx, y = by;
        if ((flags & 16) && batch >= 8) xcd_order(ntiles, batch, x, y);
        xcd_items[2 * (by * ntiles + bx)] = x;
        xcd_items[2 * (by * ntiles + bx) + 1] = y;
      }
  }
  return 0;
}

int gpc_debug_gemm_form(gpc_ctx* c, int dtype, int form, int tile, int batch, int flags, int block_slots,
                        const gpc_gemm_product* p1, const gpc_gemm_product* p2, const double* ep_w, long long ep_sw,
                        const double* ep_alpha, double* colsq, int* counters, int* available) {
  if (!c) return -2;
  if (!p1 || !counters || !available || batch <= 0 || batch > 64 || form < GPC_FORM_PLAIN || form > GPC_FORM_WSQ ||
      (tile != 64 && tile != 128) || (dtype != GPC_F64 && dtype != GPC_F32) || flags > 31 || block_slots > 4096)
    FAIL(c, "gpc_debug_gemm_form: bad arguments");
  const int vec = dtype == GPC_F64 ? 2 : 4;
  const gpc_gemm_product* prods[2] = {p1, p2};
  const int nprod = form == GPC_FORM_DUAL ? 2 : 1;
  if (nprod == 2 && !p2) FAIL(c, "gpc_debug_gemm_form: the dual form takes two products");
  for (int i = 0; i < nprod; ++i)
    if (const char* e = form_product_error(*prods[i], batch, vec)) {
      c->err = std::string("gpc_debug_gemm_form: ") + e;
      return -2;
    }
  if (form == GPC_FORM_DUAL && (p1->a_kmajor || p1->b_kmajor || p2->a_kmajor || !p2->b_kmajor))
    FAIL(c, "gpc_debug_gemm_form: the dual launch is m-major x m-major beside m-major x k-major");
  if (form == GPC_FORM_COLSQ && (p1->a_kmajor || !p1->b_kmajor || p1->lower_only || !colsq))
    FAIL(c, "gpc_debug_gemm_form: colsq is m-major x k-major over all tiles and needs the colsq output");
  if (form == GPC_FORM_WSQ && (!p1->a_kmajor || !p1->b_kmajor || p1->lower_only || !colsq || !ep_w || !ep_alpha ||
                               (batch > 1 && ep_sw != 0 && ep_sw < p1->M) || ep_sw < 0 || ep_sw > (1ll << 27)))
    FAIL(c, "gpc_debug_gemm_form: wsq is k-major x k-major over all tiles and needs colsq, ep_w, ep_alpha");
  HIPCHK(c, hipSetDevice(c->device));
  return dtype == GPC_F64 ? debug_gemm_form_impl<double>(c, form, tile, batch, flags, block_slots, prods, nprod, ep_w, ep_sw,
                                                         ep_alpha, colsq, counters, available)
                          : debug_gemm_form_impl<float>(c, form, tile, batch, flags, block_slots, prods, nprod, ep_w, ep_sw,
                                                        ep_alpha, colsq, counters, available);
}

int gpc_debug_leaf(gpc_ctx* c, int dtype, const double* A, double* L, double* W, double* logdet, int* info) {
  return gpc_debug_factor(c, dtype, TILE, A, L, W, nullptr, logdet, info);
}

int gpc_debug_factor(gpc_ctx* c, int dtype, int n, const double* A, double* L, double* W, double* Ainv,
                     double* logdet, int* info) {
  if (!c) return -2;
  if (!A || n <= 0) FAIL(c, "gpc_debug_factor: bad arguments");
  HIPCHK(c, hipSetDevice(c->device));
  return dtype == GPC_F64 ? debug_factor_impl<double>(c, n, A, L, W, Ainv, logdet, info)
                          : debug_factor_impl<float>(c, n, A, L, W, Ainv, logdet, info);
}

int gpc_debug_factor_plan(gpc_ctx* c, int dtype, int npad, int nvalid, int batch, int plan, int nll_block, int flags,
                          double* A, double* W, double* T, const double* r, double* z, double* Ainv, double* logdet,
                          int* info) {
  if (!c) return -2;
  if (dtype != GPC_F64 && dtype != GPC_F32) FAIL(c, "gpc_debug_factor_plan: dtype must be GPC_F64 or GPC_F32");
  if (npad < TILE || npad % TILE != 0 || npad > 2048)
    FAIL(c, "gpc_debug_factor_plan: npad must be a multiple of 128 in 128 .. 2048");
  if (batch < 1 || batch > 16) FAIL(c, "gpc_debug_factor_plan: batch must be 1 .. 16");
  if (plan < 0 || plan > 2) FAIL(c, "gpc_debug_factor_plan: plan must be 0, 1 or 2");
  if (plan == 2 && (nll_block < TILE || nll_block % TILE != 0 || nll_block > npad))
    FAIL(c, "gpc_debug_factor_plan: nll_block must be a multiple of 128 in 128 .. npad");
  if (flags < 0 || flags > 7) FAIL(c, "gpc_debug_factor_plan: flags has bits 0 .. 2");
  if ((flags & 4) && plan != 0) FAIL(c, "gpc_debug_factor_plan: the inverse (bit 2) belongs to plan 0");
  if (nvalid < 0 || !A || !W || !T || !logdet || !info || (r && !z) || ((flags & 4) && !Ainv))
    FAIL(c, "gpc_debug_factor_plan: bad arguments");
  HIPCHK(c, hipSetDevice(c->device));
  return dtype == GPC_F64 ? debug_factor_plan_impl<double>(c, npad, nvalid, batch, plan, nll_block, flags, A, W, T, r, z,
                                                           Ainv, logdet, info)
                          : debug_factor_plan_impl<float>(c, npad, nvalid, batch, plan, nll_block, flags, A, W, T, r, z,
                                                          Ainv, logdet, info);
}

int gpc_debug_cov(gpc_ctx* c, int which, int kernel_id, int degree, int dtype, const double* hyp_cov, double kscale,
                  double sl, const double* dvec, const double* X, int N, int D, const double* Xstar, int M,
                  const double* mat, const double* vec, double* out0, double* out1, double* xs_out) {
  if (!c) return -2;
  if (!valid_kernel(kernel_id, degree) || !hyp_cov || !X || N <= 0 || D <= 0 || !out0 || which < 0 || which > 4)
    FAIL(c, "gpc_debug_cov: bad arguments");
  if (which == 1 && N > TILE) FAIL(c, "gpc_debug_cov: the small front builds one 128 x 128 leaf (N <= 128)");
  if ((which == 2 || which == 4) && (!Xstar || M <= 0 || !vec || !out1))
    FAIL(c, "gpc_debug_cov: cross needs X*, alpha and both outputs");
  if (which == 3 && (!mat || !vec || !out1)) FAIL(c, "gpc_debug_cov: trace needs T, a and both outputs");
  HIPCHK(c, hipSetDevice(c->device));
  CovDesc cd;
  cd.kind = kernel_id;
  cd.degree = degree;
  cd.D = D;
  cd.cov_N = cov_count_of(kernel_id, D);
  return dtype == GPC_F64
             ? debug_cov_impl<double>(c, which, cd, hyp_cov, kscale, sl, dvec, X, N, Xstar, M, mat, vec, out0, out1, xs_out)
             : debug_cov_impl<float>(c, which, cd, hyp_cov, kscale, sl, dvec, X, N, Xstar, M, mat, vec, out0, out1, xs_out);
}

int gpc_debug_block_gram(gpc_ctx* c, int dtype, int n, int M, int Dp, const double* Y, const double* Z, int diag_only,
                         double* out) {
  if (!c) return -2;
  if (!Y || !out || n <= 0 || M <= 0 || Dp <= 0 || (dtype != GPC_F64 && dtype != GPC_F32))
    FAIL(c, "gpc_debug_block_gram: bad arguments");
  HIPCHK(c, hipSetDevice(c->device));
  return dtype == GPC_F64 ? debug_block_gram_impl<double>(c, n, M, Dp, Y, Z, diag_only != 0, out)
                          : debug_block_gram_impl<float>(c, n, M, Dp, Y, Z, diag_only != 0, out);
}

int gpc_debug_blas1(gpc_ctx* c, int which, int dtype, const int* ip, const double* const* in, const long long* in_n,
                    double* const* out, const long long* out_n) {
  if (!c) return -2;
  if (!ip || !in || !in_n || !out || !out_n || (dtype != GPC_F64 && dtype != GPC_F32))
    FAIL(c, "gpc_debug_blas1: bad arguments");
  HIPCHK(c, hipSetDevice(c->device));
  return dtype == GPC_F64 ? debug_blas1_impl<double>(c, which, ip, in, in_n, out, out_n)
                          : debug_blas1_impl<float>(c, which, ip, in, in_n, out, out_n);
}

int gpc_debug_hess_contract(gpc_ctx* c, int kernel_id, int degree, int dtype, const double* hyp_cov, const double* X, int N,
                            int D, const double* xstar, int M, const double* alpha, const double* Q, double* out_alpha,
                            double* out_q) {
  if (!c) return -2;
  if (!valid_kernel(kernel_id, degree) || !hyp_cov || !X || N <= 0 || D <= 0 || !xstar || M <= 0 || !alpha || !out_alpha ||
      (Q && !out_q) || (dtype != GPC_F64 && dtype != GPC_F32))
    FAIL(c, "gpc_debug_hess_contract: bad arguments");
  if ((kernel_id == K_MATERN || kernel_id == K_MATERN_ISO) && degree == 1)
    FAIL(c, "gpc_debug_hess_contract: the Matern kernel of degree 1 has no second derivative with respect to x*");
  HIPCHK(c, hipSetDevice(c->device));
  CovDesc cd;
  cd.kind = kernel_id;
  cd.degree = degree;
  cd.D = D;
  cd.cov_N = cov_count_of(kernel_id, D);
  return dtype == GPC_F64 ? debug_hess_impl<double>(c, cd, hyp_cov, X, N, xstar, M, alpha, Q, out_alpha, out_q)
                          : debug_hess_impl<float>(c, cd, hyp_cov, X, N, xstar, M, alpha, Q, out_alpha, out_q);
}

int gpc_debug_hyp_cross(gpc_ctx* c, int kernel_id, int degree, const double* hyp_cov, const double* X, int N, int D,
                        const double* xstar, int M, const double* alpha, const double* W, int P, const double* Q,
                        double* out) {
  if (!c) return -2;
  if (!valid_kernel(kernel_id, degree) || !hyp_cov || !X || N <= 0 || D <= 0 || !xstar || M <= 0 || !alpha || !W || P <= 0 ||
      !out)
    FAIL(c, "gpc_debug_hyp_cross: bad arguments");
  if ((kernel_id == K_MATERN || kernel_id == K_MATERN_ISO) && degree == 1)
// ... 246 lines not shown
```

### gpyreg_amd/csrc/plan.h

```cpp
#pragma once
#include "blas1.h"
#include "gemm.h"
#include "leaf.h"

#include <algorithm>

namespace gpc {

#ifdef GPC_EXPERIMENTS
struct PlanRecorder {
  struct Op {
    int kind;
    GemmArgs g;
    bool akm, bkm;
    int off;
  };
  std::vector<Op> ops;
  bool unsupported = false;
};
#endif

template <typename T>
struct Factor {
#ifdef GPC_EXPERIMENTS
  PlanRecorder* rec = nullptr;
#else
  static constexpr void* rec = nullptr;
#endif
  hipStream_t st;
  int batch;
  int npad;
  int nvalid = 1 << 30;
  T* A;
  T* W;
  T* Tm;
  long long sA, sW, sT;
  double* logdet;
  int* info;
  int* ctr = nullptr;
  int ctr_cap = 0, ctr_used = 0;
  hipStream_t side = nullptr;
  hipEvent_t* evs = nullptr;
  int nev = 0, ev_used = 0;
  int defer_min = 0;
  const unsigned short* reserve = nullptr;
  struct QueueCheck {
    int* slot;
    int ntiles, batch;
  };
  std::vector<QueueCheck>* qlog = nullptr;
#ifdef GPC_EXPERIMENTS
  bool reserve_all = false;
  int reserve_min = 64;
  int reserved_small_bt = 128;
#else
  static constexpr bool reserve_all = false;
  static constexpr int reserve_min = 64, reserved_small_bt = 128;
#endif
  bool dual_launch = g_dual_launch;
  bool stable = false;
  hipEvent_t ev_tail = nullptr;
  int tail_row0 = 1 << 30;
  void need_rows(int hi) {
    if (ev_tail && hi > tail_row0) {
      chk(hipStreamWaitEvent(st, ev_tail, 0));
      ev_tail = nullptr;
    }
  }
  double flops = 0;
  int launches = 0;
  hipError_t err = hipSuccess;

  T* blk(T* base, int r, int c) const { return base + (size_t)r * npad + c; }

  GemmArgs make_args(T* C, long long sC, const T* Aop, long long sAop, const T* Bop, long long sBop, int M, int N,
                     int K, double alpha, int beta, int klo, int khi, int lower) {
    GemmArgs g;
    g.A = Aop;
    g.B = Bop;
    g.C = C;
    g.sA = sAop;
    g.sB = sBop;
    g.sC = sC;
    g.lda = g.ldb = g.ldc = npad;
    g.M = M;
    g.N = N;
    g.K = K;
    g.alpha = alpha;
    g.beta = beta;
    g.klo = klo;
    g.khi = khi;
    g.lower_only = lower;
    g.tiles_n = N / TILE;
    flops += gemm_flops(g, batch);
    return g;
  }

  void gemm(T* C, long long sC, const T* Aop, long long sAop, const T* Bop, long long sBop, int M,
            int N, int K, bool akm, bool bkm, double alpha, int beta, int klo, int khi, int lower,
            hipStream_t on = nullptr, const unsigned short* rsv = nullptr) {
    GemmArgs g;
    g.A = Aop;
    g.B = Bop;
    g.C = C;
    g.sA = sAop;
    g.sB = sBop;
    g.sC = sC;
    g.lda = g.ldb = g.ldc = npad;
    g.M = M;
    g.N = N;
    g.K = K;
    g.alpha = alpha;
    g.beta = beta;
    g.klo = klo;
    g.khi = khi;
    g.lower_only = lower;
    g.tiles_n = N / TILE;
    flops += gemm_flops(g, batch);
    ++launches;
#ifdef GPC_EXPERIMENTS
    if (rec) {
      rec->ops.push_back({0, g, akm, bkm, 0});
      return;
    }
#endif
    int* slot = nullptr;
    const long long tm = M / TILE, tn = N / TILE;
    const long long blocks128 = (lower ? tm * (tm + 1) / 2 : tm * tn) * batch;
    if (!rsv && reserve_all && reserve && blocks128 >= reserve_min) rsv = reserve;
    const bool persistent = rsv || (blocks128 >= g_small_launch_blocks && blocks128 > g_block_slots - g_persist_spare);
    if (persistent && ctr && ctr_used + CTR_STRIDE <= ctr_cap) {
      slot = ctr + ctr_used;
      ctr_used += CTR_STRIDE;
      if (qlog) qlog->push_back({slot, (int)(lower ? tm * (tm + 1) / 2 : tm * tn), batch});
    }
    hipError_t e = launch_gemm<T>(on ? on : st, g, akm, bkm, batch, 0, slot, rsv, reserved_small_bt);
    if (e != hipSuccess && err == hipSuccess) err = e;
  }

  void chk(hipError_t e) {
    if (e != hipSuccess && err == hipSuccess) err = e;
  }

  void potrf_inv(int off, int n, bool need_inv, bool keep_L) {
    keep_L = keep_L || stable;
    if (n == TILE) {
#ifdef GPC_EXPERIMENTS
      if (rec) {
        if (stable) rec->unsupported = true;
        rec->ops.push_back({1, GemmArgs{}, false, false, off});
        flops += (2.0 / 3.0) * TILE * (double)TILE * TILE * batch;
        ++launches;
        return;
      }
#endif
      need_rows(off + TILE);
      launch_leaf<T>(st, batch, blk(A, off, off), sA, npad, blk(W, off, off), sW, npad, off, logdet, info,
                     std::max(0, std::min(TILE, nvalid - off)), stable);
      flops += (2.0 / 3.0) * TILE * (double)TILE * TILE * batch;
      ++launches;
      return;
    }
    const int q = n / TILE;
    const int n1 = (q / 2) * TILE, n2 = n - n1;
    const int o1 = off, o2 = off + n1;
    potrf_inv(o1, n1, true, keep_L);
    need_rows(o2 + n2);
    gemm(blk(Tm, o2, o1), sT, blk(A, o2, o1), sA, blk(W, o1, o1), sW, n2, n1, n1, false, false, 1.0,
         0, KLO_ZERO, KHI_COL, 0);
    if (stable) {
      gemm(blk(A, o2, o1), sA, blk(Tm, o2, o1), sT, blk(A, o1, o1), sA, n2, n1, n1, false, false, -1.0, 1, KLO_ZERO,
           KHI_COL, 0);
      gemm(blk(Tm, o2, o1), sT, blk(A, o2, o1), sA, blk(W, o1, o1), sW, n2, n1, n1, false, false, 1.0, 1, KLO_ZERO,
           KHI_COL, 0);
    }
    const bool defer = need_inv && side && defer_min > 0 && n >= defer_min && ev_used + 2 <= nev;
    bool u_done = false;
    {
      GemmArgs gs = make_args(blk(A, o2, o2), sA, blk(Tm, o2, o1), sT, blk(Tm, o2, o1), sT, n2, n2, n1, -1.0, 1,
                              KLO_ZERO, KHI_FULL, 1);
      const long long syrk_tiles = (long long)(n2 / TILE) * (n2 / TILE + 1) / 2 * batch;
      if (need_inv && !defer && dual_launch && !rec && gemm_is_small(gs, batch) && !(reserve_all && syrk_tiles >= reserve_min)) {
        GemmArgs gu = make_args(blk(A, o2, o1), sA, blk(Tm, o2, o1), sT, blk(W, o1, o1), sW, n2, n1, n1, 1.0, 0,
                                KLO_COL, KHI_FULL, 0);
        if (gemm_is_small(gu, batch)) {
          hipError_t e = launch_gemm_dual_small<T>(st, gs, gu, batch);
          if (e != hipSuccess && err == hipSuccess) err = e;
          ++launches;
          u_done = true;
        } else {
          flops -= gemm_flops(gu, batch);
        }
      }
      if (!u_done) {
        flops -= gemm_flops(gs, batch);
        gemm(blk(A, o2, o2), sA, blk(Tm, o2, o1), sT, blk(Tm, o2, o1), sT, n2, n2, n1, false, false, -1.0, 1,
             KLO_ZERO, KHI_FULL, 1);
      }
    }
    hipEvent_t ev_join = nullptr;
    if (defer) {
      hipEvent_t ev_fork = evs[ev_used++];
      ev_join = evs[ev_used++];
      chk(hipEventRecord(ev_fork, st));
      chk(hipStreamWaitEvent(side, ev_fork, 0));
      gemm(blk(A, o2, o1), sA, blk(Tm, o2, o1), sT, blk(W, o1, o1), sW, n2, n1, n1, false, true, 1.0, 0,
           KLO_COL, KHI_FULL, 0, side, reserve);
      chk(hipEventRecord(ev_join, side));
    }
    potrf_inv(o2, n2, need_inv, keep_L);
    if (need_inv) {
      if (defer)
        chk(hipStreamWaitEvent(st, ev_join, 0));
      else if (!u_done)
        gemm(blk(A, o2, o1), sA, blk(Tm, o2, o1), sT, blk(W, o1, o1), sW, n2, n1, n1, false, true, 1.0, 0,
             KLO_COL, KHI_FULL, 0);
      gemm(blk(W, o2, o1), sW, blk(W, o2, o2), sW, blk(A, o2, o1), sA, n2, n1, n2, false, true, -1.0,
           0, KLO_ZERO, KHI_ROW, 0);
    }
#ifdef GPC_EXPERIMENTS
    if (keep_L && rec) rec->unsupported = true;
#endif
    if (keep_L && !rec) {
      dim3 grid((n1 + 64 * MM<T>::VEC - 1) / (64 * MM<T>::VEC), n2 / 32, batch), block(64, 4);
      hipLaunchKernelGGL((rect_copy_kernel<T>), grid, block, 0, st, (const T*)blk(Tm, o2, o1), sT, npad,
                         blk(A, o2, o1), sA, npad, n2, n1);
      ++launches;
    }
  }

  int nll_block = 0;

  void trsm_nll(int r0, int m, int c0, int n) {
    if (n <= nll_block) {
      gemm(blk(Tm, r0, c0), sT, blk(A, r0, c0), sA, blk(W, c0, c0), sW, m, n, n, false, false, 1.0, 0, KLO_ZERO,
           KHI_COL, 0);
      if (stable) {
        gemm(blk(A, r0, c0), sA, blk(Tm, r0, c0), sT, blk(A, c0, c0), sA, m, n, n, false, false, -1.0, 1, KLO_ZERO,
             KHI_COL, 0);
        gemm(blk(Tm, r0, c0), sT, blk(A, r0, c0), sA, blk(W, c0, c0), sW, m, n, n, false, false, 1.0, 1, KLO_ZERO,
             KHI_COL, 0);
      }
      return;
    }
    const int q = n / TILE;
    const int n1 = (q / 2) * TILE, n2 = n - n1;
    trsm_nll(r0, m, c0, n1);
    gemm(blk(A, r0, c0 + n1), sA, blk(Tm, r0, c0), sT, blk(Tm, c0 + n1, c0), sT, m, n2, n1, false, false, -1.0, 1,
         KLO_ZERO, KHI_FULL, 0);
    trsm_nll(r0, m, c0 + n1, n2);
  }

  void potrf_nll(int off, int n) {
    if (n <= nll_block || n == TILE) {
      potrf_inv(off, n, true, false);
      return;
    }
    const int q = n / TILE;
    const int n1 = (q / 2) * TILE, n2 = n - n1;
    const int o1 = off, o2 = off + n1;
    potrf_nll(o1, n1);
    need_rows(o2 + n2);
    trsm_nll(o2, n2, o1, n1);
    gemm(blk(A, o2, o2), sA, blk(Tm, o2, o1), sT, blk(Tm, o2, o1), sT, n2, n2, n1, false, false, -1.0, 1, KLO_ZERO,
         KHI_FULL, 1);
    potrf_nll(o2, n2);
  }

  void forward_solve_nll(int off, int n, double* r, double* z) {
    if (n <= nll_block || n == TILE) {
      hipLaunchKernelGGL((trmv_kernel<T>), dim3(n / 4, batch), dim3(256), 0, st, (const T*)W, sW, npad,
                         (const double*)r, npad, z, off);
      ++launches;
      return;
    }
    const int q = n / TILE;
    const int n1 = (q / 2) * TILE, n2 = n - n1;
    forward_solve_nll(off, n1, r, z);
    hipLaunchKernelGGL((gemv_sub_kernel<T>), dim3(n2 / 4, batch), dim3(256), 0, st, (const T*)Tm, sT, npad,
                       (const double*)z, r, npad, off + n1, off, n1);
    ++launches;
    forward_solve_nll(off + n1, n2, r, z);
  }

#ifdef GPC_EXPERIMENTS
  int rl_panel = 0;
  bool rl_lookahead = true;

  void potrf_rl() {
    const int P = rl_panel;
    hipEvent_t pending = nullptr;
    for (int o = 0; o < npad; o += P) {
      const int nb = std::min(P, npad - o), rest = npad - o - nb;
      need_rows(o + nb);
      potrf_inv(o, nb, true, false);
      if (rest == 0) break;
      need_rows(npad);
      gemm(blk(Tm, o + nb, o), sT, blk(A, o + nb, o), sA, blk(W, o, o), sW, rest, nb, nb, false, false, 1.0, 0,
           KLO_ZERO, KHI_COL, 0);
      const int nb2 = std::min(P, rest), rest2 = rest - nb2;
      if (pending) {
        chk(hipStreamWaitEvent(st, pending, 0));
        pending = nullptr;
      }
      gemm(blk(A, o + nb, o + nb), sA, blk(Tm, o + nb, o), sT, blk(Tm, o + nb, o), sT, rest, nb2, nb, false, false,
           -1.0, 1, KLO_ZERO, KHI_FULL, 0);
      if (rest2 > 0) {
        const int o2 = o + nb + nb2;
        const bool ahead = rl_lookahead && side && reserve && ev_used + 2 <= nev;
        if (ahead) {
          hipEvent_t ev_fork = evs[ev_used++];
          pending = evs[ev_used++];
          chk(hipEventRecord(ev_fork, st));
          chk(hipStreamWaitEvent(side, ev_fork, 0));
        }
        gemm(blk(A, o2, o2), sA, blk(Tm, o2, o), sT, blk(Tm, o2, o), sT, rest2, rest2, nb, false, false, -1.0, 1,
             KLO_ZERO, KHI_FULL, 1, ahead ? side : nullptr, ahead ? reserve : nullptr);
        if (ahead) chk(hipEventRecord(pending, side));
      }
    }
    if (pending) chk(hipStreamWaitEvent(st, pending, 0));
  }

  void forward_solve_rl(double* r, double* z) {
    const int P = rl_panel;
    for (int o = 0; o < npad; o += P) {
      const int nb = std::min(P, npad - o), rest = npad - o - nb;
      hipLaunchKernelGGL((trmv_kernel<T>), dim3(nb / 4, batch), dim3(256), 0, st, (const T*)W, sW, npad,
                         (const double*)r, npad, z, o);
      ++launches;
      if (rest > 0) {
        hipLaunchKernelGGL((gemv_sub_kernel<T>), dim3(rest / 4, batch), dim3(256), 0, st, (const T*)Tm, sT, npad,
                           (const double*)z, r, npad, o + nb, o, nb);
        ++launches;
      }
    }
  }

#endif

  bool low_regs = false;
  void forward_solve(int off, int n, bool need_inv, double* r, double* z) {
    if (need_inv || n == TILE) {
      if (low_regs && off == 0 && n == npad)
        hipLaunchKernelGGL((trmv_low_kernel<T>), dim3(n / 16, batch), dim3(256), 0, st, (const T*)W, sW, npad,
                           (const double*)r, npad, z);
      else
        hipLaunchKernelGGL((trmv_kernel<T>), dim3(n / 4, batch), dim3(256), 0, st, (const T*)W, sW, npad,
                           (const double*)r, npad, z, off);
      ++launches;
      return;
    }
    const int q = n / TILE;
    const int n1 = (q / 2) * TILE, n2 = n - n1;
    forward_solve(off, n1, true, r, z);
    hipLaunchKernelGGL((gemv_sub_kernel<T>), dim3(n2 / 4, batch), dim3(256), 0, st, (const T*)Tm, sT, npad,
                       (const double*)z, r, npad, off + n1, off, n1);
    ++launches;
    forward_solve(off + n1, n2, need_inv, r, z);
  }

  void lauum(T* out, long long sOut) {
    gemm(out, sOut, W, sW, W, sW, npad, npad, npad, true, true, 1.0, 0, KLO_ROW, KHI_FULL, 1);
  }
};

}
```

### include/gpcore.h

```cpp
#ifndef GPCORE_H
#define GPCORE_H

#ifdef __cplusplus
extern "C" {
#endif

typedef struct gpc_ctx gpc_ctx;
typedef struct gpc_post gpc_post;

enum { GPC_K_SE = 0, GPC_K_MATERN = 1, GPC_K_RQ = 2, GPC_K_SE_ISO = 3, GPC_K_MATERN_ISO = 4 };
enum { GPC_F64 = 0, GPC_F32 = 1 };

int gpc_create(int device, gpc_ctx** out);
void gpc_destroy(gpc_ctx* ctx);
const char* gpc_last_error(const gpc_ctx* ctx);
const char* gpc_device_info(gpc_ctx* ctx);

int gpc_set_data(gpc_ctx* ctx, const double* X, const double* y, int N, int D);

int gpc_cov_count(int kernel_id, int D);
int gpc_max_n(int dtype);

int gpc_kernel(gpc_ctx* ctx, int kernel_id, int degree, const double* hyp_cov,
               const double* X, int N, int D, const double* Xstar, int M, int diag,
// ... 83 lines not shown
int gpc_lookahead_batch(gpc_post* post, const double* xr, int Mr, const double* xc, int Mc, const double* w,
                        int w_per_sample, const double* noise, int q, int* idx, double* gain);

int gpc_quad(gpc_post* post, const double* mu, const double* sigma, int M, int compute_var,
             double* zalpha, double* zKz);

int gpc_quad_grad(gpc_post* post, const double* mu, const double* sigma, int M, int compute_var,
                  double* zalpha, double* zKz, double* dza_dmu, double* dza_dsigma, double* dzkz_dmu,
                  double* dzkz_dsigma);

int gpc_quad_cov(gpc_post* post, const double* mu, const double* sigma, int M, double* zalpha, double* cov);

int gpc_quad_mix(gpc_post* post, const double* mu, const double* sigma, const double* w, int M, int compute_var,
                 int compute_grad, double* zalpha, double* zbkzb, double* gw, double* zq, double* dza_dmu,
                 double* dza_dsigma, double* dzq_dmu, double* dzq_dsigma, double* dgw_dmu, double* dgw_dsigma);

int gpc_cv(gpc_post* post, int F, const int* fold_ptr, const int* fold_idx, double* dmu, double* s2, double* quad,
           double* logdet, int* info);

int gpc_last_timing(gpc_ctx* ctx, double* ms_total, double* ms_factor);
int gpc_last_lauum_timing(gpc_ctx* ctx, double* ms, double* flops);
int gpc_set_option(gpc_ctx* ctx, const char* name, int value);
int gpc_get_option(gpc_ctx* ctx, const char* name, int* value);
int gpc_mfma_peak(gpc_ctx* ctx, int dtype, double* tflops, double* cycles_per_mfma,
                  double* clock_ghz);

int gpc_debug_gemm(gpc_ctx* ctx, int dtype, int M, int N, int K, int a_kmajor,
                   int b_kmajor, double alpha, int beta, int klo, int khi,
                   int lower_only, const double* A, const double* B, double* C);
int gpc_debug_leaf(gpc_ctx* ctx, int dtype, const double* A, double* L, double* W,
                   double* logdet, int* info);
int gpc_debug_factor(gpc_ctx* ctx, int dtype, int n, const double* A, double* L,
                     double* W, double* Ainv, double* logdet, int* info);
int gpc_debug_factor_plan(gpc_ctx* ctx, int dtype, int npad, int nvalid, int batch, int plan, int nll_block, int flags,
                          double* A, double* W, double* T, const double* r, double* z, double* Ainv, double* logdet,
                          int* info);
int gpc_debug_cov(gpc_ctx* ctx, int which, int kernel_id, int degree, int dtype, const double* hyp_cov,
                  double kscale, double sl, const double* dvec, const double* X, int N, int D,
                  const double* Xstar, int M, const double* mat, const double* vec, double* out0,
                  double* out1, double* xs_out);

int gpc_debug_blas1(gpc_ctx* ctx, int which, int dtype, const int* ip, const double* const* in, const long long* in_n,
                    double* const* out, const long long* out_n);

int gpc_debug_remove_panel(gpc_ctx* ctx, int dtype, int k, const double* D, const double* Vp, double* Theta,
                           double* Dnew);

int gpc_debug_remove_apply(gpc_ctx* ctx, int dtype, int which, int a, int n, int k, const double* Theta, double* P,
                           double* Cr);

int gpc_debug_block_gram(gpc_ctx* ctx, int dtype, int n, int M, int Dp, const double* Y, const double* Z, int diag_only,
                         double* out);

int gpc_debug_hess_contract(gpc_ctx* ctx, int kernel_id, int degree, int dtype, const double* hyp_cov, const double* X,
                            int N, int D, const double* xstar, int M, const double* alpha, const double* Q,
                            double* out_alpha, double* out_q);

int gpc_debug_hyp_cross(gpc_ctx* ctx, int kernel_id, int degree, const double* hyp_cov, const double* X, int N, int D,
                        const double* xstar, int M, const double* alpha, const double* W, int P, const double* Q,
                        double* out);

int gpc_debug_nll_plane(gpc_ctx* ctx, int kernel_id, int degree, const double* hyp_cov, const double* X, int N, int D,
                        int p, const double* alpha, const double* Q, double* plane, double* u, double* g);

int gpc_debug_nll_d2(gpc_ctx* ctx, int kernel_id, int degree, const double* hyp_cov, const double* X, int N, int D,
                     const double* alpha, const double* Q, double* out);

int gpc_debug_nll_gram(gpc_ctx* ctx, int npad, int P, const double* planes, double* out);

int gpc_debug_cv_trace(gpc_ctx* ctx, int kernel_id, int degree, const double* hyp_cov, const double* X, int N, int D,
                       const double* M, const double* alpha, const double* beta, double* gsum, double* diagG);

int gpc_debug_cv_weights(gpc_ctx* ctx, int N, int loss, const double* alpha, const double* q, const double* weights,
                         double* c, double* b);

int gpc_debug_workspace_hash(gpc_ctx* ctx, int dtype, int which, int sample, unsigned long long* out);

int gpc_debug_chunk_plan(int S, unsigned long long per, unsigned long long shared, unsigned long long budget,
                         int clamp_to_one);
int gpc_debug_scratch_bytes(const char* name, int dtype, const int* dims, int ndims, unsigned long long* per,
                            unsigned long long* shared, int* misaligned);
int gpc_debug_gemm_queues(int ntiles, int batch, int flags, int tiles_m, int tiles_n, int klo, int khi, int lower_only,
                          int* q_total, int* q_items, int* tile_ij, int* xcd_items);

typedef struct gpc_gemm_product {
  int M, N, K;
  int a_kmajor, b_kmajor;
  int beta, klo, khi, lower_only;
  int lda, ldb, ldc;
  long long off_a, off_b, off_c;
  long long s_a, s_b, s_c;
  long long size_a, size_b, size_c;
  double alpha;
  const double* A;
  const double* B;
  double* C;
} gpc_gemm_product;
enum { GPC_FORM_PLAIN = 0, GPC_FORM_PERSIST = 1, GPC_FORM_PERSIST_RESERVED = 2, GPC_FORM_DUAL = 3, GPC_FORM_COLSQ = 4,
       GPC_FORM_WSQ = 5 };
int gpc_debug_gemm_form(gpc_ctx* ctx, int dtype, int form, int tile, int batch, int flags, int block_slots,
                        const gpc_gemm_product* p1, const gpc_gemm_product* p2, const double* ep_w, long long ep_sw,
                        const double* ep_alpha, double* colsq, int* counters, int* available);

int gpc_set_data_gobs(gpc_ctx* ctx, const double* X, const double* y, int N, int D, const double* Xg, const double* dy,
                      int Ng);
int gpc_posterior_batch_gobs(gpc_ctx* ctx, int kernel_id, int degree, int dtype, int S, const double* hyp_cov,
                             const double* m, const double* sn2, gpc_post** post, double* nlz, double* sn2_mult,
                             int* L_chol, int* info);
int gpc_nll_batch_gobs(gpc_ctx* ctx, int kernel_id, int degree, int dtype, int S, const double* hyp_cov,
                       const double* m, const double* sn2, double* nlz, double* sn2_mult, int* L_chol, int* info);
int gpc_predict_gobs(gpc_post* post, const double* xstar, int M, double* fmu, double* fs2);
int gpc_debug_gobs_cov(gpc_ctx* ctx, int kernel_id, int degree, const double* hyp_cov, const double* X, int N, int D,
                       const double* Xg, int Ng, double* out);
int gpc_debug_gobs_cross(gpc_ctx* ctx, int kernel_id, int degree, const double* hyp_cov, const double* X, int N, int D,
                         const double* Xg, int Ng, const double* xstar, int M, const double* alpha, double* out,
                         double* colsum);
#ifdef GPC_EXPERIMENTS
int gpc_debug_dag(int npad, int plan, int nll_blk, int small_tiles, int* counts, int* tasks_out,
                  double* alpha_out, int* succ_out, int cap_tasks, int cap_edges);

#endif

#ifdef __cplusplus
}
#endif
#endif
```

Baseline: 843.6.

## Skip zero MFMA fragments in triangular GEMM tiles of blocked Cholesky

Adds a TRI mode to the fp64 128-tile GEMM that issues only the MFMAs and fragment loads that touch nonzero parts of triangular operands. Head and tail k-slabs use compile-time fragment masks, and lower-only diagonal tiles compute and store only the lower fragments. Fragment rows and columns are interleaved across waves so the skipped work is spread evenly. The TRSM, SYRK and LAUUM call sites in the factorisation plan pass the triangle kind, gated by a tri_skip flag. The cost is more kernel instantiations and more intricate scheduling barriers, with some risk of register pressure or a worse MFMA/LDS interleave.

```diff
diff --git a/gpyreg_amd/_lib.py b/gpyreg_amd/_lib.py
--- a/gpyreg_amd/_lib.py
+++ b/gpyreg_amd/_lib.py
@@ -130,6 +130,8 @@
     "gpc_debug_chunk_plan": (C.c_int, [C.c_int, C.c_ulonglong, C.c_ulonglong, C.c_ulonglong, C.c_int]),
     "gpc_debug_scratch_bytes": (C.c_int, [C.c_char_p, C.c_int, _ip, C.c_int, _vp, _vp, _ip]),
     "gpc_debug_gemm_queues": (C.c_int, [C.c_int] * 8 + [_ip] * 4),
+    "gpc_debug_tri_masks": (C.c_int, [C.c_int] * 3 + [_ip] * 4),
+    "gpc_debug_tri_usable": (C.c_int, [C.c_int] * 11),
     "gpc_debug_gemm_form": (
         C.c_int,
         [_vp, C.c_int, C.c_int, C.c_int, C.c_int, C.c_int, C.c_int, _vp, _vp, _dp, C.c_longlong, _dp, _dp, _ip, _ip],
@@ -1235,6 +1237,29 @@
     return queues, q_total, tiles, xcd
 
 
+TRI_A_FIRST, TRI_A_LAST, TRI_B_FIRST, TRI_B_LAST, TRI_DIAG_LOWER = 1, 2, 3, 4, 8
+TRI_FLAGS_SHIFT = 8
+
+
+def tri_masks(tri, diag_tile, slab):
+    lib = load()
+    rows, cols = np.zeros((4, 4), dtype=np.int32), np.zeros((4, 4), dtype=np.int32)
+    issued, stored = np.zeros((4, 4, 4), dtype=np.int32), np.zeros((4, 4, 4), dtype=np.int32)
+    rc = lib.gpc_debug_tri_masks(int(tri), int(bool(diag_tile)), int(slab), rows.ctypes.data, cols.ctypes.data,
+                                 issued.ctypes.data, stored.ctypes.data)
+    if rc != 0:
+        raise RuntimeError(f"gpc_debug_tri_masks failed (rc={rc})")
+    return rows, cols, issued, stored
+
+
+def tri_usable(tri, a_kmajor, b_kmajor, klo, khi, lower_only, M, N, K, tile=128, dtype=F64):
+    rc = load().gpc_debug_tri_usable(int(dtype), int(tile), int(bool(a_kmajor)), int(bool(b_kmajor)), int(klo), int(khi),
+                                     int(bool(lower_only)), int(M), int(N), int(K), int(tri))
+    if rc < 0:
+        raise RuntimeError(f"gpc_debug_tri_usable failed (rc={rc})")
+    return rc
+
+
 _contexts = {}
 
 
diff --git a/gpyreg_amd/csrc/gemm.h b/gpyreg_amd/csrc/gemm.h
--- a/gpyreg_amd/csrc/gemm.h
+++ b/gpyreg_amd/csrc/gemm.h
@@ -19,6 +19,46 @@
 
 enum { KLO_ZERO = 0, KLO_ROW = 1, KLO_COL = 2 };
 enum { KHI_FULL = 0, KHI_ROW = 1, KHI_COL = 2 };
+enum { TRI_NONE = 0, TRI_A_FIRST = 1, TRI_A_LAST = 2, TRI_B_FIRST = 3, TRI_B_LAST = 4, TRI_KIND = 7, TRI_DIAG_LOWER = 8 };
+
+__host__ __device__ constexpr int tri_active(int kind, int s) {
+  return (kind == TRI_A_FIRST || kind == TRI_B_FIRST) ? s / 2 + 1 : (kind == TRI_A_LAST || kind == TRI_B_LAST) ? 4 - s / 2 : 4;
+}
+__host__ __device__ constexpr int tri_frag(int w, int i) { return 2 * i + w; }
+template <int MRM, int MRN, int I0, int I1, int J0, int J1, bool LOW = false>
+struct FragMask {
+  static constexpr bool ALL = I0 == 0 && I1 == MRM && J0 == 0 && J1 == MRN && !LOW;
+  static constexpr bool a(int i) { return i >= I0 && i < I1; }
+  static constexpr bool b(int j) { return j >= J0 && j < J1; }
+  static constexpr bool m(int i, int j) { return a(i) && b(j) && (!LOW || i >= j); }
+  static constexpr int NA = I1 - I0, NB = J1 - J0;
+  static constexpr int count() {
+    int n = 0;
+    for (int i = 0; i < MRM; ++i)
+      for (int j = 0; j < MRN; ++j) n += m(i, j) ? 1 : 0;
+    return n;
+  }
+  static constexpr int NM = count();
+};
+template <int KIND, int N, int MR>
+using TriMask = std::conditional_t<
+    KIND == TRI_A_FIRST, FragMask<MR, MR, 0, N, 0, MR>,
+    std::conditional_t<KIND == TRI_A_LAST, FragMask<MR, MR, MR - N, MR, 0, MR>,
+                       std::conditional_t<KIND == TRI_B_FIRST, FragMask<MR, MR, 0, MR, 0, N>, FragMask<MR, MR, 0, MR, MR - N, MR>>>>;
+
+template <int KD>
+inline bool tri_mask_m(int n, int i, int j) {
+  return n == 1 ? TriMask<KD, 1, 4>::m(i, j) : n == 2 ? TriMask<KD, 2, 4>::m(i, j) : n == 3 ? TriMask<KD, 3, 4>::m(i, j) : true;
+}
+inline bool tri_issued(int tri, bool diag_tile, int s, int i, int j) {
+  if ((tri & TRI_DIAG_LOWER) && diag_tile) return FragMask<4, 4, 0, 4, 0, 4, true>::m(i, j);
+  const int kind = tri & TRI_KIND, n = tri_active(kind, s);
+  return kind == TRI_A_FIRST ? tri_mask_m<TRI_A_FIRST>(n, i, j) : kind == TRI_A_LAST ? tri_mask_m<TRI_A_LAST>(n, i, j)
+       : kind == TRI_B_FIRST ? tri_mask_m<TRI_B_FIRST>(n, i, j) : kind == TRI_B_LAST ? tri_mask_m<TRI_B_LAST>(n, i, j) : true;
+}
+inline bool tri_stored(int tri, bool diag_tile, int wr, int wc, int i, int j) {
+  return !((tri & TRI_DIAG_LOWER) && diag_tile) || tri_frag(wr, i) >= tri_frag(wc, j);
+}
 
 struct GemmArgs {
   const void* A;
@@ -35,6 +75,7 @@
   const unsigned short* rsv = nullptr;
   int* ctr = nullptr;
   int ntiles = 0, batch = 0;
+  int tri = TRI_NONE;
   double* colsq = nullptr;
   const double* ep_w = nullptr;
   long long ep_sw = 0;
@@ -177,8 +218,20 @@
 #else
 #define TILE_TS(k) do { } while (0)
 #endif
-template <typename T, bool AKM, bool BKM, int BT, int NW, int HO = 0, int EPI = 0, int BTN = BT>
+template <int TRI, int WT>
+__device__ __forceinline__ int frag_org(int base, int w, int i) {
+  if constexpr (TRI)
+    return base + tri_frag(w, i) * 16;
+  else
+    return base + w * WT + i * 16;
+}
+template <typename T, bool AKM, bool BKM, int BT, int NW, int HO = 0, int EPI = 0, int BTN = BT, int TRI = TRI_NONE>
 __device__ __forceinline__ void gemm_tile(const GemmArgs& g, const int bx, const int by, T* __restrict__ smem) {
+  static_assert(TRI == TRI_NONE || (TRI >= TRI_A_FIRST && TRI <= TRI_B_LAST) || TRI == TRI_DIAG_LOWER ||
+                    TRI == (TRI_A_FIRST | TRI_DIAG_LOWER),
+                "an instantiation holds the paths of ONE launch kind (all of them in one kernel: spills in the k-loop)");
+  static_assert(!TRI || (sizeof(T) == 8 && BT == 128 && BTN == BT && NW == 4 && EPI == 0 && HO == 0),
+                "zero skipping: fp64 128-tiles of 2 x 2 waves; the column-sum epilogues keep contiguous ownership");
 #ifdef GPC_TILE_TRACE
   long long _ts = wall_clock64();
   if (HO && threadIdx.x == 0) atomicAdd(&g_tile_trace[BT == 64][3], 1ull);
@@ -205,6 +258,11 @@
   int k1 = g.khi == KHI_ROW ? m128 + TILE : (g.khi == KHI_COL ? n128 + TILE : g.K);
   if (k1 > g.K) k1 = g.K;
   const int nk = (k1 - k0) / BKT_v<T>;
+  constexpr int TKIND = TRI & TRI_KIND;
+  constexpr bool TRI_HEAD = TKIND == TRI_A_FIRST || TKIND == TRI_B_FIRST, TRI_TAIL = TKIND == TRI_A_LAST || TKIND == TRI_B_LAST;
+  constexpr bool TRI_DIAG = (TRI & TRI_DIAG_LOWER) != 0;
+  bool tdiag = false;
+  if constexpr (TRI_DIAG) tdiag = g.lower_only && ti == tj;
 
   const T* __restrict__ A = reinterpret_cast<const T*>(g.A) + (size_t)by * g.sA;
   const T* __restrict__ B = reinterpret_cast<const T*>(g.B) + (size_t)by * g.sB;
@@ -260,86 +318,167 @@
     __syncthreads();
     TILE_TS(0);
 
+    using FULL = FragMask<MRM, MRN, 0, MRM, 0, MRN>;
     T af[2][MRM], bf[2][MRN];
-    auto load_frags = [&](int set, const T* a_s, const T* b_s, int kk) {
-#pragma unroll
-      for (int i = 0; i < MRM; ++i) af[set][i] = frag<T, AKM, BT>(a_s, wr * WTM + i * 16, kk, lane);
-#pragma unroll
-      for (int j = 0; j < MRN; ++j) bf[set][j] = frag<T, BKM, BTN>(b_s, wc * WTN + j * 16, kk, lane);
+    auto load_frags = [&](auto mask_c, int set, const T* a_s, const T* b_s, int kk) {
+      using M = decltype(mask_c);
+#pragma unroll
+      for (int i = 0; i < MRM; ++i)
+        if (M::ALL || M::a(i)) af[set][i] = frag<T, AKM, BT>(a_s, frag_org<TRI, WTM>(0, wr, i), kk, lane);
+#pragma unroll
+      for (int j = 0; j < MRN; ++j)
+        if (M::ALL || M::b(j)) bf[set][j] = frag<T, BKM, BTN>(b_s, frag_org<TRI, WTN>(0, wc, j), kk, lane);
     };
-    auto mfmas = [&](int set) {
+    auto mfmas = [&](auto mask_c, int set) {
+      using M = decltype(mask_c);
 #pragma unroll
       for (int i = 0; i < MRM; ++i)
 #pragma unroll
-        for (int j = 0; j < MRN; ++j) acc[i][j] = MM<T>::mma(af[set][i], bf[set][j], acc[i][j]);
+        for (int j = 0; j < MRN; ++j)
+          if (M::ALL || M::m(i, j)) acc[i][j] = MM<T>::mma(af[set][i], bf[set][j], acc[i][j]);
     };
     constexpr int NMEM = NVA + NVB;
-    constexpr int PER = (MRM * MRN) / NMEM;
-    constexpr int REM = MRM * MRN - PER * NMEM;
-    static_assert(PER >= 1, "interleave pattern");
+    static_assert((MRM * MRN) / NMEM >= 1, "interleave pattern");
     constexpr int KS = BKT_v<T> / 4;
     static_assert(KS >= 4 && KS % 2 == 0, "fragment sets alternate per k-step and wrap per slab");
-    auto slab = [&](auto cur_c, auto wr_c, auto ld_c) {
+    auto slab = [&](auto cur_c, auto wr_c, auto ld_c, auto mask_c, auto next_c) {
       constexpr int CUR = decltype(cur_c)::value;
       constexpr bool WR = decltype(wr_c)::value, LD = decltype(ld_c)::value;
+      using M = decltype(mask_c);
+      using MN = decltype(next_c);
+      constexpr int NM = M::NM;
+      constexpr int PER = NM / NMEM;
+      constexpr int REM = NM - PER * NMEM;
       const T* a_s = smem + CUR * STG;
       const T* b_s = a_s + OPSZA;
       T* a_n = smem + (CUR ^ 1) * STG;
 #pragma unroll
       for (int ks = 0; ks < KS - 2; ++ks) {
-        load_frags((ks + 1) & 1, a_s, b_s, 4 * (ks + 1));
-        mfmas(ks & 1);
-        __builtin_amdgcn_sched_group_barrier(0x100, MRM + MRN, 0);
-        __builtin_amdgcn_sched_group_barrier(0x008, MRM * MRN, 0);
-      }
-      load_frags(1, a_s, b_s, 4 * (KS - 1));
-      mfmas(0);
+        load_frags(M{}, (ks + 1) & 1, a_s, b_s, 4 * (ks + 1));
+        mfmas(M{}, ks & 1);
+        __builtin_amdgcn_sched_group_barrier(0x100, M::NA + M::NB, 0);
+        __builtin_amdgcn_sched_group_barrier(0x008, NM, 0);
+      }
+      load_frags(M{}, 1, a_s, b_s, 4 * (KS - 1));
+      mfmas(M{}, 0);
       if constexpr (WR) {
         r2s<T, AKM, BT, NT>(a_n, ra, t);
         r2s<T, BKM, BTN, NT>(a_n + OPSZA, rb, t);
       }
-      __builtin_amdgcn_sched_group_barrier(0x100, MRM + MRN, 0);
+      __builtin_amdgcn_sched_group_barrier(0x100, M::NA + M::NB, 0);
 #pragma unroll
       for (int q = 0; q < NMEM; ++q) {
-        __builtin_amdgcn_sched_group_barrier(0x008, PER, 0);
+        if constexpr (PER >= 1)
+          __builtin_amdgcn_sched_group_barrier(0x008, PER, 0);
+        else if (q < REM)
+          __builtin_amdgcn_sched_group_barrier(0x008, 1, 0);
         if constexpr (WR) __builtin_amdgcn_sched_group_barrier(0x200, 1, 0);
       }
-      if constexpr (REM > 0) __builtin_amdgcn_sched_group_barrier(0x008, REM, 0);
+      if constexpr (PER >= 1 && REM > 0) __builtin_amdgcn_sched_group_barrier(0x008, REM, 0);
       __syncthreads();
       if constexpr (LD) {
         next_slab();
         g2r<T, AKM, BT, NT, AUX>(ra, rsa, ua, psa, toa);
         g2r<T, BKM, BTN, NT, AUX>(rb, rsb, ub, psb, tob);
       }
-      if constexpr (WR) load_frags(0, a_n, a_n + OPSZA, 0);
-      mfmas(1);
-      if constexpr (WR) __builtin_amdgcn_sched_group_barrier(0x100, MRM + MRN, 0);
+      if constexpr (WR) load_frags(MN{}, 0, a_n, a_n + OPSZA, 0);
+      mfmas(M{}, 1);
+      if constexpr (WR) __builtin_amdgcn_sched_group_barrier(0x100, MN::NA + MN::NB, 0);
 #pragma unroll
       for (int q = 0; q < NMEM; ++q) {
-        __builtin_amdgcn_sched_group_barrier(0x008, PER, 0);
+        if constexpr (PER >= 1)
+          __builtin_amdgcn_sched_group_barrier(0x008, PER, 0);
+        else if (q < REM)
+          __builtin_amdgcn_sched_group_barrier(0x008, 1, 0);
         if constexpr (LD) __builtin_amdgcn_sched_group_barrier(0x020, 1, 0);
       }
-      if constexpr (REM > 0) __builtin_amdgcn_sched_group_barrier(0x008, REM, 0);
+      if constexpr (PER >= 1 && REM > 0) __builtin_amdgcn_sched_group_barrier(0x008, REM, 0);
     };
     using I0 = std::integral_constant<int, 0>;
     using I1 = std::integral_constant<int, 1>;
-    load_frags(0, smem, smem + OPSZA, 0);
+    using YES = std::true_type;
+    using NO = std::false_type;
+    load_frags(FULL{}, 0, smem, smem + OPSZA, 0);
     int it = 0;
-    for (; it + 3 < nk; it += 2) {
-      slab(I0{}, std::true_type{}, std::true_type{});
-      slab(I1{}, std::true_type{}, std::true_type{});
-      if constexpr (TWO_LEVEL) {
-#pragma unroll
-        for (int i = 0; i < MRM; ++i)
-#pragma unroll
-          for (int j = 0; j < MRN; ++j) {
-            acc2[i][j] += acc[i][j];
-            acc[i][j] = acc_t{0, 0, 0, 0};
-          }
-      }
-    }
-    slab(I0{}, std::true_type{}, std::false_type{});
-    slab(I1{}, std::false_type{}, std::false_type{});
+    if constexpr (TRI) {
+      auto tri_head = [&](auto kind_c) {
+        constexpr int KD = decltype(kind_c)::value;
+        using M1 = TriMask<KD, 1, MRM>;
+        using M2 = TriMask<KD, 2, MRM>;
+        using M3 = TriMask<KD, 3, MRM>;
+        static_assert(tri_active(KD, 0) == 1 && tri_active(KD, 1) == 1 && tri_active(KD, 2) == 2 && tri_active(KD, 3) == 2 &&
+                      tri_active(KD, 4) == 3 && tri_active(KD, 5) == 3 && tri_active(KD, 6) == 4 && tri_active(KD, 7) == 4);
+        slab(I0{}, YES{}, YES{}, M1{}, M1{});
+        slab(I1{}, YES{}, YES{}, M1{}, M2{});
+        slab(I0{}, YES{}, YES{}, M2{}, M2{});
+        slab(I1{}, YES{}, YES{}, M2{}, M3{});
+        slab(I0{}, YES{}, YES{}, M3{}, M3{});
+        slab(I1{}, YES{}, YES{}, M3{}, FULL{});
+      };
+      auto tri_tail = [&](auto kind_c) {
+        constexpr int KD = decltype(kind_c)::value;
+        using M1 = TriMask<KD, 1, MRM>;
+        using M2 = TriMask<KD, 2, MRM>;
+        using M3 = TriMask<KD, 3, MRM>;
+        static_assert(tri_active(KD, 0) == 4 && tri_active(KD, 1) == 4 && tri_active(KD, 2) == 3 && tri_active(KD, 3) == 3 &&
+                      tri_active(KD, 4) == 2 && tri_active(KD, 5) == 2 && tri_active(KD, 6) == 1 && tri_active(KD, 7) == 1);
+        slab(I0{}, YES{}, YES{}, M3{}, M3{});
+        slab(I1{}, YES{}, YES{}, M3{}, M2{});
+        slab(I0{}, YES{}, YES{}, M2{}, M2{});
+        slab(I1{}, YES{}, YES{}, M2{}, M1{});
+        slab(I0{}, YES{}, NO{}, M1{}, M1{});
+        slab(I1{}, NO{}, NO{}, M1{}, M1{});
+      };
+      auto tri_diag = [&](auto low_c) {
+        using LOWM = decltype(low_c);
+        for (; it + 3 < nk; it += 2) {
+          slab(I0{}, YES{}, YES{}, LOWM{}, LOWM{});
+          slab(I1{}, YES{}, YES{}, LOWM{}, LOWM{});
+        }
+        slab(I0{}, YES{}, NO{}, LOWM{}, LOWM{});
+        slab(I1{}, NO{}, NO{}, LOWM{}, LOWM{});
+      };
+      bool done = false;
+      if constexpr (TRI_DIAG) {
+        if (tdiag) {
+          tri_diag(FragMask<MRM, MRN, 0, MRM, 0, MRN, true>{});
+          done = true;
+        }
+      }
+      if (!done) {
+        if constexpr (TRI_HEAD) {
+          tri_head(std::integral_constant<int, TKIND>{});
+          it = 6;
+        }
+        const int stop = TRI_TAIL ? nk - 6 : nk - 2;
+        for (; it < stop; it += 2) {
+          slab(I0{}, YES{}, YES{}, FULL{}, FULL{});
+          slab(I1{}, YES{}, YES{}, FULL{}, FULL{});
+        }
+        if constexpr (TRI_TAIL) {
+          tri_tail(std::integral_constant<int, TKIND>{});
+        } else {
+          slab(I0{}, YES{}, NO{}, FULL{}, FULL{});
+          slab(I1{}, NO{}, NO{}, FULL{}, FULL{});
+        }
+      }
+    } else {
+      for (; it + 3 < nk; it += 2) {
+        slab(I0{}, YES{}, YES{}, FULL{}, FULL{});
+        slab(I1{}, YES{}, YES{}, FULL{}, FULL{});
+        if constexpr (TWO_LEVEL) {
+#pragma unroll
+          for (int i = 0; i < MRM; ++i)
+#pragma unroll
+            for (int j = 0; j < MRN; ++j) {
+              acc2[i][j] += acc[i][j];
+              acc[i][j] = acc_t{0, 0, 0, 0};
+            }
+        }
+      }
+      slab(I0{}, YES{}, NO{}, FULL{}, FULL{});
+      slab(I1{}, NO{}, NO{}, FULL{}, FULL{});
+    }
   }
 
   TILE_TS(1);
@@ -435,8 +574,10 @@
       for (int j = 0; j < MRN; ++j)
 #pragma unroll
         for (int r = 0; r < 4; ++r) {
-          const int row = m0 + wr * WTM + i * 16 + MM<T>::row_of(lane, r);
-          const int col = n0 + wc * WTN + j * 16 + (lane & 15);
+          if constexpr (TRI_DIAG)
+            if (tdiag && tri_frag(wr, i) < tri_frag(wc, j)) continue;
+          const int row = frag_org<TRI, WTM>(m0, wr, i) + MM<T>::row_of(lane, r);
+          const int col = frag_org<TRI, WTN>(n0, wc, j) + (lane & 15);
           if constexpr (HO == 1)
             old[j][r] = __hip_atomic_load(&C[(size_t)row * g.ldc + col], __ATOMIC_RELAXED, __HIP_MEMORY_SCOPE_AGENT);
           else
@@ -447,8 +588,10 @@
     for (int j = 0; j < MRN; ++j)
 #pragma unroll
       for (int r = 0; r < 4; ++r) {
-        const int row = m0 + wr * WTM + i * 16 + MM<T>::row_of(lane, r);
-        const int col = n0 + wc * WTN + j * 16 + (lane & 15);
+        if constexpr (TRI_DIAG)
+          if (tdiag && tri_frag(wr, i) < tri_frag(wc, j)) continue;
+        const int row = frag_org<TRI, WTM>(m0, wr, i) + MM<T>::row_of(lane, r);
+        const int col = frag_org<TRI, WTN>(n0, wc, j) + (lane & 15);
         T v;
         if constexpr (TWO_LEVEL)
           v = alpha * (acc[i][j][r] + acc2[i][j][r]);
@@ -464,14 +607,14 @@
   TILE_TS(2);
 }
 
-template <typename T, bool AKM, bool BKM, int BT, int NW, int EPI = 0, int BTN = BT>
+template <typename T, bool AKM, bool BKM, int BT, int NW, int EPI = 0, int BTN = BT, int TRI = TRI_NONE>
 __global__ __launch_bounds__(64 * NW, NW / 2) void gemm_kernel(GemmArgs g) {
   __shared__ __attribute__((aligned(16))) T smem[2 * (opsz_of<T>(BT) + opsz_of<T>(BTN))];
   int bx = blockIdx.x, by = blockIdx.y;
   if ((g.flags & 16) && gridDim.y >= 8) {
     xcd_order((int)gridDim.x, (int)gridDim.y, bx, by);
   }
-  gemm_tile<T, AKM, BKM, BT, NW, 0, EPI, BTN>(g, bx, by, smem);
+  gemm_tile<T, AKM, BKM, BT, NW, 0, EPI, BTN, TRI>(g, bx, by, smem);
 }
 
 template <typename T, bool A1, bool B1, bool A2, bool B2, int BT, int NW>
@@ -485,7 +628,7 @@
     gemm_tile<T, A2, B2, BT, NW>(g2, bx - n1, by, smem);
 }
 
-template <typename T, bool AKM, bool BKM, int BT, int NW, int EPI = 0>
+template <typename T, bool AKM, bool BKM, int BT, int NW, int EPI = 0, int TRI = TRI_NONE>
 __global__ __launch_bounds__(64 * NW, NW / 2) void gemm_persist_kernel(GemmArgs g) {
   __shared__ __attribute__((aligned(16))) T smem[4 * opsz_of<T>(BT)];
   __shared__ int next_tile;
@@ -498,7 +641,7 @@
       const int idx = __builtin_amdgcn_readfirstlane(next_tile);
       __syncthreads();
       if (idx >= total) break;
-      gemm_tile<T, AKM, BKM, BT, NW, 0, EPI>(g, idx / g.batch, idx % g.batch, smem);
+      gemm_tile<T, AKM, BKM, BT, NW, 0, EPI, BT, TRI>(g, idx / g.batch, idx % g.batch, smem);
     }
     return;
   }
@@ -527,7 +670,7 @@
       if (idx >= total) break;
       const int ntq = total / nsq;
       const int sq = idx / ntq, tq = idx - sq * ntq;
-      gemm_tile<T, AKM, BKM, BT, NW, 0, EPI>(g, cls + tq * nclass, smp + NQ * sq, smem);
+      gemm_tile<T, AKM, BKM, BT, NW, 0, EPI, BT, TRI>(g, cls + tq * nclass, smp + NQ * sq, smem);
     }
   }
 }
@@ -562,6 +705,51 @@
 inline int g_persist_spare = 0;
 inline long long g_gemm_launches = 0;
 inline int g_block_slots = 512;
+template <typename T, int BT, int NW>
+inline int tri_usable(const GemmArgs& g, bool akm, bool bkm) {
+  if constexpr (sizeof(T) != 8 || BT != 128 || NW != 4) {
+    return TRI_NONE;
+  } else {
+    const int kind = g.tri & TRI_KIND;
+    const bool diag = (g.tri & TRI_DIAG_LOWER) && g.lower_only;
+    if (akm && bkm) return (kind == TRI_A_FIRST && g.klo == KLO_ROW) ? (kind | (diag ? (int)TRI_DIAG_LOWER : 0)) : (int)TRI_NONE;
+    if (!akm && bkm) {
+      if (kind == TRI_A_LAST && g.khi == KHI_ROW && g.K >= g.M) return kind;
+      if (kind == TRI_B_FIRST && g.klo == KLO_COL) return kind;
+      return TRI_NONE;
+    }
+    if (!akm && !bkm) {
+      if (kind == TRI_B_LAST && g.khi == KHI_COL && g.K >= g.N) return kind;
+      if (kind == TRI_NONE && diag) return TRI_DIAG_LOWER;
+    }
+    return TRI_NONE;
+  }
+}
+template <typename T, int BT, int NW>
+inline bool launch_gemm_tri(bool persist, dim3 grid, dim3 block, hipStream_t st, const GemmArgs& g, bool akm, bool bkm) {
+  if constexpr (sizeof(T) == 8 && BT == 128 && NW == 4) {
+#define GPC_TRI_LAUNCH(AKM, BKM, TRI)                                                                        \
+  case TRI:                                                                                                  \
+    if (akm != AKM || bkm != BKM) return false;                                                              \
+    if (persist)                                                                                             \
+      hipLaunchKernelGGL((gemm_persist_kernel<T, AKM, BKM, BT, NW, 0, TRI>), grid, block, 0, st, g);         \
+    else                                                                                                     \
+      hipLaunchKernelGGL((gemm_kernel<T, AKM, BKM, BT, NW, 0, BT, TRI>), grid, block, 0, st, g);             \
+    return true;
+    switch (g.tri) {
+      GPC_TRI_LAUNCH(true, true, TRI_A_FIRST)
+      GPC_TRI_LAUNCH(true, true, TRI_A_FIRST | TRI_DIAG_LOWER)
+      GPC_TRI_LAUNCH(false, true, TRI_A_LAST)
+      GPC_TRI_LAUNCH(false, true, TRI_B_FIRST)
+      GPC_TRI_LAUNCH(false, false, TRI_B_LAST)
+      GPC_TRI_LAUNCH(false, false, TRI_DIAG_LOWER)
+      default:
+        return false;
+    }
+#undef GPC_TRI_LAUNCH
+  }
+  return false;
+}
 template <typename T, int BT, int NW>
 inline hipError_t launch_gemm_bt(hipStream_t st, GemmArgs g, bool akm, bool bkm, int batch, int* ctr = nullptr,
                                  const unsigned short* reserve = nullptr) {
@@ -575,11 +763,14 @@
   g.ntiles = ntiles;
   g.batch = batch;
   g.ctr = ctr;
+  g.tri = tri_usable<T, BT, NW>(g, akm, bkm);
   const unsigned dyn = 0u;
   const int cap = (BT == 128 ? g_block_slots : 2 * g_block_slots) - g_persist_spare;
   g.rsv = reserve;
   if (ctr && (BT == 128 || reserve) && cap > 0 && ((long long)ntiles * batch > cap || reserve)) {
     dim3 grid(reserve ? (BT == 128 ? cap + 96 : cap) : cap), block(64 * NW);
+    if (g.tri && launch_gemm_tri<T, BT, NW>(true, grid, block, st, g, akm, bkm)) return hipGetLastError();
+    g.tri = TRI_NONE;
     if (!akm && !bkm)
       hipLaunchKernelGGL((gemm_persist_kernel<T, false, false, BT, NW>), grid, block, dyn, st, g);
     else if (!akm && bkm)
@@ -591,6 +782,8 @@
     return hipGetLastError();
   }
   dim3 grid(ntiles, batch), block(64 * NW);
+  if (g.tri && launch_gemm_tri<T, BT, NW>(false, grid, block, st, g, akm, bkm)) return hipGetLastError();
+  g.tri = TRI_NONE;
   if (!akm && !bkm)
     hipLaunchKernelGGL((gemm_kernel<T, false, false, BT, NW>), grid, block, dyn, st, g);
   else if (!akm && bkm)
diff --git a/gpyreg_amd/csrc/gpcore.hip b/gpyreg_amd/csrc/gpcore.hip
--- a/gpyreg_amd/csrc/gpcore.hip
+++ b/gpyreg_amd/csrc/gpcore.hip
@@ -397,6 +397,7 @@
   bool cu_map_ok = false;
   DevBuf rsv_tbl;
   int nll_block = -1;
+  int tri_skip = 1;
   int solves_beside_lauum = 1;
 #ifdef GPC_EXPERIMENTS
   int rl_panel = 0;
@@ -944,6 +945,7 @@
     F.info = d_info;
     F.nvalid = N;
     F.stable = stable || c->stable;
+    F.tri_skip = c->tri_skip != 0;
     if ((defer_node > 0 || use_rl) && !c->capturing && gpc::g_persist_spare >= 0) {
       F.side = c->sst[gidx];
       F.evs = c->dev_ev[gidx];
@@ -1051,7 +1053,7 @@
       }
       if (!dag_has_lauum) {
         if (!c->capturing) HIPCHK(c, hipEventRecord(c->ev_l0[gidx], st));
-        F.lauum(Tc, sM);
+        F.lauum(Tc, sM, !kmode());
         if (!c->capturing) {
           HIPCHK(c, hipEventRecord(c->ev_l1[gidx], st));
           lauum_n[gidx] = n;
@@ -3903,7 +3905,8 @@
                          const double* ep_alpha, double* colsq, int* counters, int* available) {
   HookMem mem;
   GemmGlobalsGuard guard;
-  if (flags >= 0) gpc::g_gemm_flags = flags;
+  if (flags >= 0) gpc::g_gemm_flags = flags & 0xff;
+  const int tri = flags >= 0 ? (flags >> 8) & 15 : (int)TRI_NONE;
   if (block_slots > 0) {
     gpc::g_block_slots = block_slots;
     gpc::g_persist_spare = 0;
@@ -3954,6 +3957,7 @@
     a.klo = p.klo;
     a.khi = p.khi;
     a.lower_only = p.lower_only ? 1 : 0;
+    a.tri = tri;
   }
   int* ctr = nullptr;
   HIPCHK(c, mem.get(reinterpret_cast<void**>(&ctr), CTR_STRIDE * sizeof(int)));
@@ -4114,6 +4118,7 @@
   F.logdet = dld;
   F.info = dinfo;
   F.stable = (flags & 1) != 0;
+  F.tri_skip = c->tri_skip != 0;
   const bool keep_L = (flags & 2) != 0;
   if (plan == 2) {
     F.nll_block = nll_block;
@@ -7367,6 +7372,7 @@
     {"leaf_fault", nullptr, GPC_SET(gpc::g_leaf_fault = v != 0)},
     {"nll_block", GPC_GET(c->nll_block), GPC_SET(c->nll_block = v < 0 ? -1 : (v == 0 ? 0 : tile_multiple(v)))},
     {"solves_beside_lauum", GPC_GET(c->solves_beside_lauum), GPC_SET(c->solves_beside_lauum = v != 0)},
+    {"tri_skip", GPC_GET(c->tri_skip), GPC_SET(c->tri_skip = v != 0)},
     {"stable", GPC_GET(c->stable), GPC_SET(c->stable = v != 0)},
     {"small_path", GPC_GET(c->small_path), GPC_SET(c->small_path = v != 0)},
     {"check_queues", GPC_GET(c->check_queues), GPC_SET(c->check_queues = v != 0)},
@@ -7603,12 +7609,42 @@
   return 0;
 }
 
+int gpc_debug_tri_masks(int tri, int diag_tile, int slab, int* frag_rows, int* frag_cols, int* issued, int* stored) {
+  const int kind = tri & TRI_KIND;
+  if (tri < 0 || tri > 15 || kind > TRI_B_LAST || slab < 0 || slab > 7 || !frag_rows || !frag_cols || !issued || !stored) return -2;
+  for (int w = 0; w < 4; ++w) {
+    const int wr = w / 2, wc = w % 2;
+    for (int i = 0; i < 4; ++i) {
+      frag_rows[w * 4 + i] = tri_frag(wr, i);
+      frag_cols[w * 4 + i] = tri_frag(wc, i);
+      for (int j = 0; j < 4; ++j) {
+        issued[(w * 4 + i) * 4 + j] = tri_issued(tri, diag_tile != 0, slab, i, j) ? 1 : 0;
+        stored[(w * 4 + i) * 4 + j] = tri_stored(tri, diag_tile != 0, wr, wc, i, j) ? 1 : 0;
+      }
+    }
+  }
+  return 0;
+}
+
+int gpc_debug_tri_usable(int dtype, int tile, int a_kmajor, int b_kmajor, int klo, int khi, int lower_only, int M, int N,
+                         int K, int tri) {
+  if ((dtype != GPC_F64 && dtype != GPC_F32) || (tile != 64 && tile != 128) || tri < 0 || tri > 15) return -2;
+  GemmArgs g;
+  g.M = M, g.N = N, g.K = K;
+  g.klo = klo, g.khi = khi, g.lower_only = lower_only ? 1 : 0;
+  g.tri = tri;
+  const bool akm = a_kmajor != 0, bkm = b_kmajor != 0;
+  if (dtype == GPC_F64) return tile == 128 ? tri_usable<double, 128, 4>(g, akm, bkm) : tri_usable<double, 64, 4>(g, akm, bkm);
+  return tile == 128 ? tri_usable<float, 128, 4>(g, akm, bkm) : tri_usable<float, 64, 4>(g, akm, bkm);
+}
+
 int gpc_debug_gemm_form(gpc_ctx* c, int dtype, int form, int tile, int batch, int flags, int block_slots,
                         const gpc_gemm_product* p1, const gpc_gemm_product* p2, const double* ep_w, long long ep_sw,
                         const double* ep_alpha, double* colsq, int* counters, int* available) {
   if (!c) return -2;
   if (!p1 || !counters || !available || batch <= 0 || batch > 64 || form < GPC_FORM_PLAIN || form > GPC_FORM_WSQ ||
-      (tile != 64 && tile != 128) || (dtype != GPC_F64 && dtype != GPC_F32) || flags > 31 || block_slots > 4096)
+      (tile != 64 && tile != 128) || (dtype != GPC_F64 && dtype != GPC_F32) || (flags >= 0 && ((flags & 0xff) > 31 || (flags >> 8) > 15)) ||
+      block_slots > 4096)
     FAIL(c, "gpc_debug_gemm_form: bad arguments");
   const int vec = dtype == GPC_F64 ? 2 : 4;
   const gpc_gemm_product* prods[2] = {p1, p2};
@@ -7651,8 +7687,8 @@
                           int* info) {
   if (!c) return -2;
   if (dtype != GPC_F64 && dtype != GPC_F32) FAIL(c, "gpc_debug_factor_plan: dtype must be GPC_F64 or GPC_F32");
-  if (npad < TILE || npad % TILE != 0 || npad > 2048)
-    FAIL(c, "gpc_debug_factor_plan: npad must be a multiple of 128 in 128 .. 2048");
+  if (npad < TILE || npad % TILE != 0 || (npad > 2048 && npad != 2304))
+    FAIL(c, "gpc_debug_factor_plan: npad must be a multiple of 128 in 128 .. 2048, or 2304");
   if (batch < 1 || batch > 16) FAIL(c, "gpc_debug_factor_plan: batch must be 1 .. 16");
   if (plan < 0 || plan > 2) FAIL(c, "gpc_debug_factor_plan: plan must be 0, 1 or 2");
   if (plan == 2 && (nll_block < TILE || nll_block % TILE != 0 || nll_block > npad))
diff --git a/gpyreg_amd/csrc/plan.h b/gpyreg_amd/csrc/plan.h
--- a/gpyreg_amd/csrc/plan.h
+++ b/gpyreg_amd/csrc/plan.h
@@ -67,6 +67,8 @@
       ev_tail = nullptr;
     }
   }
+  bool tri_skip = false;
+  int tri(int what) const { return tri_skip ? what : (int)TRI_NONE; }
   double flops = 0;
   int launches = 0;
   hipError_t err = hipSuccess;
@@ -98,8 +100,9 @@
 
   void gemm(T* C, long long sC, const T* Aop, long long sAop, const T* Bop, long long sBop, int M,
             int N, int K, bool akm, bool bkm, double alpha, int beta, int klo, int khi, int lower,
-            hipStream_t on = nullptr, const unsigned short* rsv = nullptr) {
+            hipStream_t on = nullptr, const unsigned short* rsv = nullptr, int tri_what = TRI_NONE) {
     GemmArgs g;
+    g.tri = tri(tri_what);
     g.A = Aop;
     g.B = Bop;
     g.C = C;
@@ -167,12 +170,12 @@
     potrf_inv(o1, n1, true, keep_L);
     need_rows(o2 + n2);
     gemm(blk(Tm, o2, o1), sT, blk(A, o2, o1), sA, blk(W, o1, o1), sW, n2, n1, n1, false, false, 1.0,
-         0, KLO_ZERO, KHI_COL, 0);
+         0, KLO_ZERO, KHI_COL, 0, nullptr, nullptr, TRI_B_LAST);
     if (stable) {
       gemm(blk(A, o2, o1), sA, blk(Tm, o2, o1), sT, blk(A, o1, o1), sA, n2, n1, n1, false, false, -1.0, 1, KLO_ZERO,
-           KHI_COL, 0);
+           KHI_COL, 0, nullptr, nullptr, TRI_B_LAST);
       gemm(blk(Tm, o2, o1), sT, blk(A, o2, o1), sA, blk(W, o1, o1), sW, n2, n1, n1, false, false, 1.0, 1, KLO_ZERO,
-           KHI_COL, 0);
+           KHI_COL, 0, nullptr, nullptr, TRI_B_LAST);
     }
     const bool defer = need_inv && side && defer_min > 0 && n >= defer_min && ev_used + 2 <= nev;
     bool u_done = false;
@@ -195,7 +198,7 @@
       if (!u_done) {
         flops -= gemm_flops(gs, batch);
         gemm(blk(A, o2, o2), sA, blk(Tm, o2, o1), sT, blk(Tm, o2, o1), sT, n2, n2, n1, false, false, -1.0, 1,
-             KLO_ZERO, KHI_FULL, 1);
+             KLO_ZERO, KHI_FULL, 1, nullptr, nullptr, keep_L ? TRI_NONE : TRI_DIAG_LOWER);
       }
     }
     hipEvent_t ev_join = nullptr;
@@ -205,7 +208,7 @@
       chk(hipEventRecord(ev_fork, st));
       chk(hipStreamWaitEvent(side, ev_fork, 0));
       gemm(blk(A, o2, o1), sA, blk(Tm, o2, o1), sT, blk(W, o1, o1), sW, n2, n1, n1, false, true, 1.0, 0,
-           KLO_COL, KHI_FULL, 0, side, reserve);
+           KLO_COL, KHI_FULL, 0, side, reserve, TRI_B_FIRST);
       chk(hipEventRecord(ev_join, side));
     }
     potrf_inv(o2, n2, need_inv, keep_L);
@@ -214,9 +217,9 @@
         chk(hipStreamWaitEvent(st, ev_join, 0));
       else if (!u_done)
         gemm(blk(A, o2, o1), sA, blk(Tm, o2, o1), sT, blk(W, o1, o1), sW, n2, n1, n1, false, true, 1.0, 0,
-             KLO_COL, KHI_FULL, 0);
+             KLO_COL, KHI_FULL, 0, nullptr, nullptr, TRI_B_FIRST);
       gemm(blk(W, o2, o1), sW, blk(W, o2, o2), sW, blk(A, o2, o1), sA, n2, n1, n2, false, true, -1.0,
-           0, KLO_ZERO, KHI_ROW, 0);
+           0, KLO_ZERO, KHI_ROW, 0, nullptr, nullptr, TRI_A_LAST);
     }
 #ifdef GPC_EXPERIMENTS
     if (keep_L && rec) rec->unsupported = true;
@@ -234,12 +237,12 @@
   void trsm_nll(int r0, int m, int c0, int n) {
     if (n <= nll_block) {
       gemm(blk(Tm, r0, c0), sT, blk(A, r0, c0), sA, blk(W, c0, c0), sW, m, n, n, false, false, 1.0, 0, KLO_ZERO,
-           KHI_COL, 0);
+           KHI_COL, 0, nullptr, nullptr, TRI_B_LAST);
       if (stable) {
         gemm(blk(A, r0, c0), sA, blk(Tm, r0, c0), sT, blk(A, c0, c0), sA, m, n, n, false, false, -1.0, 1, KLO_ZERO,
-             KHI_COL, 0);
+             KHI_COL, 0, nullptr, nullptr, TRI_B_LAST);
         gemm(blk(Tm, r0, c0), sT, blk(A, r0, c0), sA, blk(W, c0, c0), sW, m, n, n, false, false, 1.0, 1, KLO_ZERO,
-             KHI_COL, 0);
+             KHI_COL, 0, nullptr, nullptr, TRI_B_LAST);
       }
       return;
     }
@@ -263,7 +266,7 @@
     need_rows(o2 + n2);
     trsm_nll(o2, n2, o1, n1);
     gemm(blk(A, o2, o2), sA, blk(Tm, o2, o1), sT, blk(Tm, o2, o1), sT, n2, n2, n1, false, false, -1.0, 1, KLO_ZERO,
-         KHI_FULL, 1);
+         KHI_FULL, 1, nullptr, nullptr, stable ? TRI_NONE : TRI_DIAG_LOWER);
     potrf_nll(o2, n2);
   }
 
@@ -360,8 +363,9 @@
     forward_solve(off + n1, n2, need_inv, r, z);
   }
 
-  void lauum(T* out, long long sOut) {
-    gemm(out, sOut, W, sW, W, sW, npad, npad, npad, true, true, 1.0, 0, KLO_ROW, KHI_FULL, 1);
+  void lauum(T* out, long long sOut, bool lower_frags_only = false) {
+    gemm(out, sOut, W, sW, W, sW, npad, npad, npad, true, true, 1.0, 0, KLO_ROW, KHI_FULL, 1, nullptr, nullptr,
+         TRI_A_FIRST | (lower_frags_only ? TRI_DIAG_LOWER : 0));
   }
 };
 
diff --git a/include/gpcore.h b/include/gpcore.h
--- a/include/gpcore.h
+++ b/include/gpcore.h
@@ -189,6 +189,9 @@
                             unsigned long long* shared, int* misaligned);
 int gpc_debug_gemm_queues(int ntiles, int batch, int flags, int tiles_m, int tiles_n, int klo, int khi, int lower_only,
                           int* q_total, int* q_items, int* tile_ij, int* xcd_items);
+int gpc_debug_tri_masks(int tri, int diag_tile, int slab, int* frag_rows, int* frag_cols, int* issued, int* stored);
+int gpc_debug_tri_usable(int dtype, int tile, int a_kmajor, int b_kmajor, int klo, int khi, int lower_only, int M, int N,
+                         int K, int tri);
 
 typedef struct gpc_gemm_product {
   int M, N, K;
```

Result: faster. 858.5, median of 6 (+1.8%).
